# rvp-group/mrhash

Measured on AMD Instinct MI355X. Metric: depth frames/sec integrated (640x480), higher is better.
Workload: dtype f32; 1 GPU; replica-room0 stand-in 640x480, single-resolution hash TSDF integrate (alloc+compact+integrate+GC per frame, replica.cfg params), frames resident in HBM; frames_per_gpu=7880, parallelism=single GPU, live_blocks_end=39984, distinct_frames=200

## Files before the change

mrhash_amd/csrc/mrh_context.h:

```cpp
#pragma once

constexpr int kPipeRing = 6;

namespace {

thread_local std::string g_create_err;

struct EvPair {
  hipEvent_t a, b;
};

struct UpSlot {
  void* h = nullptr;
  void* d = nullptr;
  size_t cap = 0;
  hipEvent_t copied = nullptr;
  bool copied_rec = false;
  uint64_t last_seq = 0;
};
struct UpRing {
  UpSlot s[3];
  int cur = -1;
  hipStream_t stream = nullptr;
  hipEvent_t last_copy = nullptr;
  bool waited[2] = {false, false};
};

template <typename T>
struct HostVec {
  T* p = nullptr;
  T* dev = nullptr;
  bool pin = true;
  size_t n = 0, cap = 0;
  size_t span = 0, head = 0;
  HostVec() = default;
  HostVec(const HostVec&) = delete;
  HostVec& operator=(const HostVec&) = delete;
  ~HostVec() { release(); }
  void release() {
    if (!p) return;
    if (dev) (void) hipHostUnregister((void*) p);
    (void) munmap((void*) ((char*) p - head), span);
    p = nullptr; dev = nullptr; cap = 0; span = 0; head = 0;
  }
  T* data() { return p; }
  const T* data() const { return p; }
  size_t size() const { return n; }
  bool empty() const { return n == 0; }
  void clear() { n = 0; }
  const T& operator[](size_t i) const { return p[i]; }
  bool pin_pending = false;
  void map_(const size_t count, const bool touch) {
    release();
    const size_t want = count + count / 8;
    const size_t bytes = ((want * sizeof(T) + (2u << 20) - 1) >> 21) << 21;
    const size_t sp = bytes + (2u << 20);
    void* m = mmap(nullptr, sp, PROT_READ | PROT_WRITE, MAP_PRIVATE | MAP_ANONYMOUS, -1, 0);
    if (m == MAP_FAILED) throw std::bad_alloc();
    char* aligned = (char*) (((uintptr_t) m + (2u << 20) - 1) & ~(uintptr_t) ((2u << 20) - 1));
    (void) madvise(aligned, bytes, MADV_HUGEPAGE);
    if (touch) for (size_t o = 0; o < bytes; o += 4096) ((volatile char*) aligned)[o] = 0;
    span = sp;
    head = (size_t) (aligned - (char*) m);
    p = (T*) aligned;
    dev = nullptr;
    cap = bytes / sizeof(T);
  }
  void register_() {
    pin_pending = false;
    void* d = nullptr;
    const size_t bytes = cap * sizeof(T);
    if (hipHostRegister((void*) p, bytes, hipHostRegisterDefault) == hipSuccess && hipHostGetDevicePointer(&d, (void*) p, 0) == hipSuccess && d) {
      dev = (T*) d;
    } else {
      (void) hipGetLastError();
      (void) hipHostUnregister((void*) p);
      (void) hipGetLastError();
      dev = nullptr;
    }
  }
  void reserve_unpinned(const size_t count) {
    if (count <= cap) return;
    map_(count, true);
    pin_pending = pin;
    n = 0;
  }
  void resize_discard(size_t count) {
    if (count > cap) {
      map_(count, pin);
      pin_pending = false;
      if (pin) register_();
    } else if (pin_pending) {
      register_();
    }
    n = count;
  }
  void assign(const T* a, const T* b) {
    resize_discard((size_t) (b - a));
    if (n) memcpy(p, a, n * sizeof(T));
  }
};

struct FrameInputs {
  Cam cam;
  const float* d_depth; const uint8_t* d_rgb;
  int depth_rows, depth_cols, rgb_rows, rgb_cols;
  struct Ring { int cur; hipEvent_t last_copy; bool waited[2]; } ring[2];
};
struct DeferredFrame {
  bool on = false;
  int n_inval = 0;
  FrameInputs in;
};

enum FrameKind {
  FRAME_SERIAL,
  FRAME_PIPELINED,
  FRAME_FUSED_MR,
  FRAME_GENERAL,
};
struct FramePlan {
  FrameKind kind = FRAME_SERIAL;
  int max_num_frames = 0;
  bool starve_now = false;
  bool starve_fused = false;
  bool starve_in_pipe = false;
  bool gc_inline = false;
  bool safe_div = false, sph = false;
  float gc_thr = 0.f;
  int set = 0, zero_set = 0;
  int ring = 0, seq = 0;
  u32 stamp = 0;
  int tiles_x = 0, n_tiles = 0;
};
struct PendingBack {
  FramePlan plan;
  Cam cam; Fast f; Lists L;
  EvPair ev;
  uint64_t report_seq;
  bool count_zombies;
};

struct PipeState {
  hipStream_t stream_front = nullptr;
  hipEvent_t ev_front[kPipeRing] = {};
  int4* ring_vis[kPipeRing] = {}; int4* ring_bbox[kPipeRing] = {}; int4* ring_cfree[kPipeRing] = {}; float* ring_zmin[kPipeRing] = {};
  u32* want_ring = nullptr;
  int* h_levels = nullptr;
  uint2* dcx[kPipeRing] = {};
  size_t npix = 0;
  uint64_t fast_frames = 0;
  uint64_t seq = 0;
  uint64_t base = 0;
  int lazy_run = 0;
  bool zombies_possible = false;
  bool front_needs_sync = false;
  static constexpr int kPendMax = 3;
  PendingBack pendq[kPendMax];
  int npend = 0;
  bool last_frame_lazy = false;
  bool flushed_since_frame = false;
  int sync_streak = 0;
  u64* d_zfused = nullptr;
  size_t zfused_n = 0;
  bool zfused_clean[2] = {false, false};
  size_t zfused_clean_npix = 0;
  int zfused_next = 0;
};

}

struct mrh_ctx {
  mrh_params p;
  int device = 0;
  hipStream_t stream = nullptr;
  struct Owned { std::vector<void*> dev, pinned; std::vector<hipEvent_t> events; } owned;
  Cam cam;
  Map map;
  Tab tab;
  bool has_camera = false;
  bool spherical = false;
  UpRing up_depth, up_rgb;
  DeferredFrame deferred;
  int defer_uploads = 1;
  hipEvent_t frame_done[8] = {};
  hipEvent_t peek_done[8] = {};
  uint64_t frame_seq = 1;
  int* h_peek = nullptr;
  void* arena[3] = {nullptr, nullptr, nullptr};
  size_t arena_cap[3] = {0, 0, 0};
  uint64_t peek_seq[8] = {};
  bool peek_enabled = false;
  const float* d_depth = nullptr;
  const uint8_t* d_rgb = nullptr;
  int depth_rows = 0, depth_cols = 0, rgb_rows = 0, rgb_cols = 0;
  u32* d_decision = nullptr;
  u64* d_zbuf = nullptr;
  size_t zbuf_n = 0;
  bool starve_fused = true;
  bool starve_serial = false;
  uint64_t n_starve_fused = 0;
  int4* d_realloc = nullptr;
  int4* d_reint = nullptr;
  int* d_flag = nullptr;
  u64* d_upd_partials = nullptr;
  u32* d_misc = nullptr;
  float* d_rcp_w = nullptr;
  Fast fast;
  int pipe = 1;
  int pipe_grid = 1024;
  int pipe_uploads = 0;
  int pipe_period = 64;
  bool pipe_always_wait = false;
  int pipe_defer = 1;
  PipeState ps;
  FramePlan plan;
  uint64_t dbg_waits = 0;
  double dbg_spin_us = 0, dbg_api_us = 0; uint64_t dbg_lazy_frames = 0;
  int4* d_cfree = nullptr;
  float* d_cloud = nullptr; size_t cloud_n = 0;
  bool fast_summaries_stale = false;
  struct Lidar {
    float* d_points = nullptr;
    const float* d_points_cur = nullptr;
    size_t points_cap = 0, num_points = 0;
    float* d_normals = nullptr; size_t normals_cap = 0, num_normals = 0;
    bool have_cloud = false;
    int layout_hint = 0;
    int row_len = 0;
    uint64_t detect_n = 0;
    int detect_len = 0, detect_age = 0;
    int patch_log2 = 4;
    u32* d_pt_counts = nullptr; u32* d_pt_offsets = nullptr; size_t pt_cap = 0;
    u32* h_sorted_report = nullptr;
    u32 sorted_seq = 0;
    void* d_rec_keys[2] = {nullptr, nullptr}; float* d_rec_vals[2] = {nullptr, nullptr}; size_t rec_cap = 0, rec_key_bytes = 0;
    void* d_sort_tmp = nullptr; size_t sort_tmp_bytes = 0;
    Scan buckets = {};
    int use_buckets = 1;
    int buckets_scratch = 0;
    bool buckets_dirty = false;
    size_t buckets_rec_cap = 0, buckets_wg_cap = 0;
    u32* d_buckets_ctr = nullptr;
    u32 buckets_seq = 0;
    size_t buckets_lds_set = 0;
  } lidar;
  size_t qt_cap = 0;
  QSum* d_qt_sums = nullptr; u32* d_qt_flags = nullptr; u32* d_qt_unc = nullptr; u64* d_qt_marks = nullptr; u64* d_qt_pos = nullptr;
  mrh_splat_seed* d_qt_parked = nullptr; mrh_qtree_leaf* d_qt_leaves = nullptr;
  mrh_splat_seed* h_qt_seeds = nullptr; size_t qt_seed_cap = 0;
  u64* h_qt_out = nullptr;
  u64* d_qt_misc = nullptr;
  int qt_literal = 0;
  uint32_t qt_last_literal = 0;
  std::vector<mrh_qtree_leaf> qt_leaves;
  uint64_t qt_n_leaves = 0;
  bool qt_leaves_on_host = true;
  int mr_fused = 1;
  bool mr_next_general = true;
  bool mr_summaries_valid = false;
  bool refill_flag_valid = false;
  int mesh_on_host = 0;
  float* d_zmin = nullptr;
  u64* d_cnt_partials = nullptr;
  int fused_grid = 2048;
  int sweep_wgs_mr = 1024;
  int sweep_wgs = 128;
  int integrate_grid = 1024;
  int low_blocks_to_allocate = 0;
  uint64_t num_blocks = 0, slots = 0, max_triangles = 0;
  uint64_t frames = 0;
  int heap_descending = 0;
  int pending = 0;
  HostVec<mrh_triangle> tris;
  std::vector<mrh_block_desc> tri_blocks;
  std::vector<uint32_t> tri_counts;
  int tri_dev_n = 0;
  const int4* d_tri_sorted = nullptr;
  const u32* d_tri_counts = nullptr;
  u64* h_mc = nullptr;
  hipEvent_t ev_mc_total = nullptr;
  u32* d_mc_recs = nullptr; size_t mc_rec_cap = 0;
  uint64_t mc_rec_fallbacks = 0;
  HostVec<double> V, C;
  HostVec<int32_t> F;
  HostVec<float> V32, C32;
  HostVec<u32> stage_ctl;
  u32 stage_epoch = 0;
  void* mesh_clean_base = nullptr;
  size_t mesh_clean_words = 0;
  bool prewarm_on = true, prewarm_done = false;
  uint64_t n_extractions = 0;
  bool f64_link = false;
  int profile = 0;
  std::vector<EvPair> ev_pool;
  std::vector<EvPair> ev_pending;
  std::vector<EvPair> ev_pending_front;
  float sum_ms = 0.f, last_ms = 0.f;
  uint64_t n_ms = 0;
  float sum_front_ms = 0.f;
  uint64_t n_front_ms = 0;
  uint64_t prev_total_updated = 0, prev_inserted = 0, prev_freed = 0, total_compact = 0;
  uint64_t last_triangles = 0;
  int census_period = 64;
  int census_force = 0;
  uint64_t frames_since_census = 0;
  bool table_dirty = false;
  u32 flags_seen = 0, flags_deferred = 0, flags_peeked = 0;
  char* d_pack = nullptr; size_t pack_cap = 0;
  mrh_triangle* d_soup = nullptr; size_t soup_cap = 0, soup_n = 0;
  int4* d_halo = nullptr; size_t halo_cap = 0, halo_upper = 0;
  u32* d_taken = nullptr;
  hipEvent_t mc_ev[4] = {};
  float last_mc_count_ms = 0.f, last_mc_emit_ms = 0.f;
  uint64_t last_mc_blocks = 0;
  bool merge_on = false;
  mrh_triangle* d_acc = nullptr; size_t acc_cap = 0, acc_n = 0;
  mrh_comm* comm = nullptr;
  char* d_xsend = nullptr; size_t xsend_cap = 0;
  char* d_xrecv = nullptr; size_t xrecv_cap = 0;
  hipEvent_t comm_ev[5] = {};
  mrh_comm_phases comm_phases = {};
  std::vector<EvPair> comm_ev_pool, comm_ev_pending;
  char* d_ray = nullptr; size_t ray_cap = 0;
  char* h_ray = nullptr; size_t h_ray_cap = 0;
  struct Normals {
    NrmTab tab = {};
    size_t cap = 0;
    u64* d_ctr = nullptr;
    u32 seq = 0;
    bool dirty = false;
    int fold = 1;
    u64* h_ctr = nullptr;
    mrh_normals_info info = {};
    bool info_pending = false;
    float* h_out = nullptr; size_t h_out_cap = 0;
  } nrm;
  std::string err;
};

static int comm_allreduce_zbuf(mrh_ctx* c, mrh::u64* buf, size_t n);
static void comm_release(mrh_ctx* c);
static bool comm_matches_sharding(const mrh_ctx* c, int* comm_rank, int* comm_world);
namespace {
int strict_point(mrh_ctx* c);
int flush_deferred(mrh_ctx* c);
void main_stream_changed_map(mrh_ctx* c) { c->ps.front_needs_sync = true; }

int fail(mrh_ctx* c, int code, const char* fmt, ...) {
  char buf[512];
  va_list ap;
  va_start(ap, fmt);
  vsnprintf(buf, sizeof buf, fmt, ap);
  va_end(ap);
  if (c) c->err = buf;
  else g_create_err = buf;
  return code;
}

#define HIP_TRY(ctx, expr)                                                                                   \
  do {                                                                                                       \
    hipError_t e__ = (expr);                                                                                 \
    if (e__ != hipSuccess) return fail(ctx, MRH_ERR_DEVICE, "%s failed: %s (%s:%d)", #expr, hipGetErrorString(e__), __FILE__, __LINE__); \
  } while (0)

template <typename T>
struct DevBuf {
  T* p = nullptr;
  DevBuf() = default;
  DevBuf(const DevBuf&) = delete;
  DevBuf& operator=(const DevBuf&) = delete;
  ~DevBuf() { if (p) (void) hipFree(p); }
  hipError_t alloc(size_t n) { return hipMalloc((void**) &p, n * sizeof(T)); }
  operator T*() const { return p; }
};

template <typename T> hipError_t own(std::vector<void*>& ledger, T*& p, const hipError_t e) {
  if (e != hipSuccess) p = nullptr; else ledger.push_back((void*) p);
  return e;
}
template <typename T> hipError_t disown(std::vector<void*>& ledger, T*& p, hipError_t (*release)(void*)) {
  const auto it = std::find(ledger.begin(), ledger.end(), (void*) p);
  const hipError_t e = !p ? hipSuccess : it == ledger.end() ? hipErrorInvalidValue : release((void*) p);
  if (it != ledger.end()) { *it = ledger.back(); ledger.pop_back(); }
  p = nullptr;
  return e;
}
template <typename T> hipError_t dev_alloc(mrh_ctx* c, T*& p, const size_t bytes) { return own(c->owned.dev, p, hipMalloc((void**) &p, bytes)); }
template <typename T> hipError_t dev_free(mrh_ctx* c, T*& p) { return disown(c->owned.dev, p, hipFree); }
template <typename T> hipError_t pinned_alloc(mrh_ctx* c, T*& p, const size_t bytes) { return own(c->owned.pinned, p, hipHostMalloc((void**) &p, bytes, hipHostMallocDefault)); }
template <typename T> hipError_t pinned_free(mrh_ctx* c, T*& p) { return disown(c->owned.pinned, p, hipHostFree); }
hipError_t event_new(mrh_ctx* c, hipEvent_t& ev, const bool timing) {
  const hipError_t e = timing ? hipEventCreate(&ev) : hipEventCreateWithFlags(&ev, hipEventDisableTiming);
  if (e != hipSuccess) ev = nullptr; else c->owned.events.push_back(ev);
  return e;
}

struct GrowMember {
  void** p; size_t bytes;
  template <typename T> GrowMember(T*& q, size_t b) : p((void**) &q), bytes(b) {}
};
int regrow_all(mrh_ctx* c, size_t& cap, const size_t cap_new, std::initializer_list<GrowMember> members, const bool sync = true) {
  cap = 0;
  if (sync) HIP_TRY(c, hipStreamSynchronize(c->stream));
  for (const GrowMember& m : members) HIP_TRY(c, dev_free(c, *m.p));
  for (const GrowMember& m : members) {
    const hipError_t e = dev_alloc(c, *m.p, m.bytes);
    if (e == hipSuccess) continue;
    for (const GrowMember& f : members) (void) dev_free(c, *f.p);
    return fail(c, MRH_ERR_DEVICE, "hipMalloc of %zu bytes failed: %s", m.bytes, hipGetErrorString(e));
  }
  cap = cap_new;
  return MRH_OK;
}
template <typename T>
int regrow(mrh_ctx* c, T*& p, size_t& cap, const size_t cap_new, const size_t bytes, const bool sync = true) {
  return cap_new <= cap ? MRH_OK : regrow_all(c, cap, cap_new, {{p, bytes}}, sync);
}
template <typename T>
int regrow_keep(mrh_ctx* c, T*& p, size_t& cap, const size_t cap_new, const size_t bytes_new, const size_t keep_bytes) {
  if (cap_new <= cap) return MRH_OK;
  T* grown = nullptr;
  HIP_TRY(c, dev_alloc(c, grown, bytes_new));
  struct Drop { mrh_ctx* c; T*& p; ~Drop() { (void) dev_free(c, p); } } drop{c, grown};
  if (p && keep_bytes) HIP_TRY(c, hipMemcpyAsync(grown, p, keep_bytes, hipMemcpyDeviceToDevice, c->stream));
  HIP_TRY(c, hipStreamSynchronize(c->stream));
  std::swap(p, grown); cap = cap_new;
  return MRH_OK;
}
template <typename T>
int regrow_pinned(mrh_ctx* c, T*& p, size_t& cap, const size_t cap_new, const size_t bytes) {
  if (cap_new <= cap) return MRH_OK;
  cap = 0;
  (void) pinned_free(c, p);
  HIP_TRY(c, pinned_alloc(c, p, bytes));
  cap = cap_new;
  return MRH_OK;
}

uint64_t next_pow2(uint64_t v) {
  uint64_t r = 1;
  while (r < v) r <<= 1;
  return r;
}

void free_all(mrh_ctx* c) {
  if (!c) return;
  (void) hipSetDevice(c->device);
  hipStream_t* streams[4] = {&c->up_depth.stream, &c->up_rgb.stream, &c->ps.stream_front, &c->stream};
  for (hipStream_t* s : streams) if (*s) (void) hipStreamSynchronize(*s);
  comm_release(c);
  for (hipEvent_t e : c->owned.events) (void) hipEventDestroy(e);
  for (void* p : c->owned.pinned) (void) hipHostFree(p);
  for (void* p : c->owned.dev) (void) hipFree(p);
  c->owned = {};
  for (hipStream_t* s : streams) if (*s) { (void) hipStreamDestroy(*s); *s = nullptr; }
}

void reset_pipe_counters(mrh_ctx* c) {
  PipeState& ps = c->ps;
  for (int i = 0; i < ps.npend; i++) if (ps.pendq[i].ev.a) c->ev_pool.push_back(ps.pendq[i].ev);
  ps.npend = 0;
  ps.fast_frames = 0;
  ps.seq = ps.base = 0;
  ps.lazy_run = 0;
  ps.zombies_possible = false;
  ps.front_needs_sync = false;
}

int init_buffers(mrh_ctx* c) {
  hipStream_t s = c->stream;
  c->mr_next_general = true;
  c->refill_flag_valid = false;
  c->mr_summaries_valid = false;
  if (c->ps.stream_front) HIP_TRY(c, hipStreamSynchronize(c->ps.stream_front));
  reset_pipe_counters(c);
  if (c->ps.h_levels) { c->ps.h_levels[0] = (int) c->num_blocks - 1; c->ps.h_levels[1] = 0; c->ps.h_levels[2] = -1; }
  if (c->ps.want_ring) HIP_TRY(c, hipMemsetAsync(c->ps.want_ring, 0, (size_t) kPipeRing * c->slots * sizeof(u32), s));
  const Tab& t = c->tab;
  k_init_table<<<1024, 256, 0, s>>>(t.keys, c->slots);
  k_init_heap<<<1024, 256, 0, s>>>(t.heap_fine, (u32) c->num_blocks, c->heap_descending);
  HIP_TRY(c, hipMemsetAsync(t.vals, 0, c->slots * sizeof(u32), s));
  HIP_TRY(c, hipMemsetAsync(t.desc_fine, 0, c->num_blocks * sizeof(int4), s));
  if (t.multi_res) HIP_TRY(c, hipMemsetAsync(t.desc_coarse, 0, c->num_blocks * 8 * sizeof(int4), s));
  HIP_TRY(c, hipMemsetAsync(t.pool, 0, c->num_blocks * (size_t) kFineBytes, s));
  int h_ctr[CTR_COUNT];
  memset(h_ctr, 0, sizeof h_ctr);
  h_ctr[CTR_HEAP_FINE] = (int) c->num_blocks - 1;
  h_ctr[CTR_HEAP_COARSE] = -1;
  HIP_TRY(c, hipMemcpyAsync(t.ctr, h_ctr, sizeof h_ctr, hipMemcpyHostToDevice, s));
  HIP_TRY(c, hipMemsetAsync(t.prof, 0, PROF_COUNT * sizeof(u64), s));
  HIP_TRY(c, hipMemsetAsync(c->d_upd_partials, 0, (size_t) c->integrate_grid * sizeof(u64), s));
  HIP_TRY(c, hipMemsetAsync(c->d_cnt_partials, 0, (size_t) 32768 * 4 * sizeof(u64), s));
  HIP_TRY(c, hipStreamSynchronize(s));
  c->frames = 0;
  c->frames_since_census = 0;
  c->table_dirty = false;
  c->flags_seen = c->flags_deferred = c->flags_peeked = 0;
  c->halo_upper = 0;
  c->prev_total_updated = c->prev_inserted = c->prev_freed = c->total_compact = 0;
  c->sum_ms = c->last_ms = 0.f;
  c->n_ms = 0;
  c->sum_front_ms = 0.f;
  c->n_front_ms = 0;
  c->tris.clear(); c->V.clear(); c->C.clear(); c->F.clear();
  c->last_triangles = 0;
  return MRH_OK;
}

int create_checks(const mrh_params* p) {
  if (p->abi_version != MRH_ABI_VERSION) return fail(nullptr, MRH_ERR_INVALID_ARG, "mrh_create: abi_version mismatch");
  if (!(p->virtual_voxel_size > 0.f)) return fail(nullptr, MRH_ERR_INVALID_ARG, "mrh_create: virtual_voxel_size must be > 0");
  if (!(p->sdf_truncation >= 0.f) || !(p->sdf_truncation_scale >= 0.f))
    return fail(nullptr, MRH_ERR_INVALID_ARG, "mrh_create: sdf_truncation and sdf_truncation_scale must be >= 0");
  if (p->voxel_extents_scale != 0 && p->voxel_extents_scale != 1)
    return fail(nullptr, MRH_ERR_UNSUPPORTED, "mrh_create: voxel_extents_scale != 1 is incoherent in the reference (vhu.cuh:90-92 vs 138-140)");
  int ndev = 0;
  if (hipGetDeviceCount(&ndev) != hipSuccess || ndev <= 0) return fail(nullptr, MRH_ERR_NO_DEVICE, "mrh_create: no HIP device visible");
  if (p->device_id < 0 || p->device_id >= ndev) return fail(nullptr, MRH_ERR_INVALID_ARG, "mrh_create: device_id %d out of range (%d devices)", p->device_id, ndev);
  if (p->shard_count > 1 && (p->shard_rank < 0 || p->shard_rank >= p->shard_count))
    return fail(nullptr, MRH_ERR_INVALID_ARG, "mrh_create: shard_rank out of range");
  return MRH_OK;
}

int size_map(mrh_ctx* c, const mrh_params* p) {
  c->p = *p;
  if (c->p.integration_weight_max == 0) c->p.integration_weight_max = 255;
  if (c->p.voxel_extents_scale == 0) c->p.voxel_extents_scale = 1;
  if (c->p.shard_count < 1) c->p.shard_count = 1;
  c->device = p->device_id;
  memset(&c->tab, 0, sizeof c->tab); memset(&c->cam, 0, sizeof c->cam); memset(&c->fast, 0, sizeof c->fast);
  HIP_TRY(c, hipSetDevice(c->device));
  HIP_TRY(c, hipStreamCreateWithFlags(&c->stream, hipStreamNonBlocking));
  size_t free_b = 0, total_b = 0;
  HIP_TRY(c, hipMemGetInfo(&free_b, &total_b));
  const double to_alloc = (double) free_b * 0.70;
  c->num_blocks = p->num_sdf_blocks ? p->num_sdf_blocks : (uint64_t) ((to_alloc * 0.70) / (12.0 * 512.0));
  if (c->num_blocks >= (1ull << 28)) c->num_blocks = (1ull << 28) - 1;
  c->max_triangles = p->max_triangles ? p->max_triangles : (uint64_t) ((to_alloc * 0.25) / 72.0);
  c->slots = std::max<uint64_t>(1024, next_pow2(p->hash_slots ? p->hash_slots : 4 * c->num_blocks));
  c->low_blocks_to_allocate = (int) ((float) c->num_blocks * 0.1f);
  c->fast.zlist_cap = (u32) c->num_blocks;
  Tab& t = c->tab;
  t.slot_mask = (u32) (c->slots - 1); t.max_probe = 512; t.cap_blocks = (u32) c->num_blocks;
  t.multi_res = p->sdf_var_threshold > 0.f ? 1u : 0u;
  Map& m = c->map;
  m.vs = p->virtual_voxel_size; m.trunc = p->sdf_truncation; m.trunc_scale = p->sdf_truncation_scale;
  m.var_threshold = p->sdf_var_threshold; m.mc_threshold = p->marching_cubes_threshold; m.min_weight_threshold = p->min_weight_threshold;
  m.weight_sample = p->integration_weight_sample & 0xFF; m.weight_max = c->p.integration_weight_max & 0xFF;
  m.shard_rank = c->p.shard_rank; m.shard_count = c->p.shard_count;
  m.shard_chunk_log2 = (p->shard_chunk_log2 > 0 && p->shard_chunk_log2 < 16) ? p->shard_chunk_log2 : 3;
  return MRH_OK;
}

int alloc_map(mrh_ctx* c) {
  Tab& t = c->tab;
  const size_t nb = c->num_blocks, list_cap = nb * (t.multi_res ? 9 : 1);
  HIP_TRY(c, dev_alloc(c, t.keys, c->slots * sizeof(u64)));                HIP_TRY(c, dev_alloc(c, t.vals, c->slots * sizeof(u32)));
  HIP_TRY(c, dev_alloc(c, t.heap_fine, (nb + 1) * sizeof(u32)));           HIP_TRY(c, dev_alloc(c, t.desc_fine, nb * sizeof(int4)));
  if (t.multi_res) {
    HIP_TRY(c, dev_alloc(c, t.heap_coarse, (nb * 8 + 9) * sizeof(u32)));   HIP_TRY(c, dev_alloc(c, t.desc_coarse, nb * 8 * sizeof(int4)));
    HIP_TRY(c, dev_alloc(c, c->d_realloc, nb * sizeof(int4)));             HIP_TRY(c, dev_alloc(c, c->d_reint, nb * sizeof(int4)));
    HIP_TRY(c, dev_alloc(c, c->fast.summary_c, nb * 8 * sizeof(uint2)));
  }
  HIP_TRY(c, dev_alloc(c, t.pool, nb * (size_t) kFineBytes));
  HIP_TRY(c, dev_alloc(c, t.compact, list_cap * sizeof(int4)));            HIP_TRY(c, dev_alloc(c, c->d_decision, list_cap * sizeof(u32)));
  HIP_TRY(c, dev_alloc(c, t.ctr, CTR_COUNT * sizeof(int)));                HIP_TRY(c, dev_alloc(c, t.prof, PROF_COUNT * sizeof(u64)));
  HIP_TRY(c, dev_alloc(c, c->d_flag, sizeof(int)));                        HIP_TRY(c, dev_alloc(c, c->d_misc, 4 * sizeof(u32)));
  HIP_TRY(c, dev_alloc(c, c->d_upd_partials, (size_t) c->integrate_grid * sizeof(u64)));
  HIP_TRY(c, dev_alloc(c, c->d_cnt_partials, (size_t) 32768 * 4 * sizeof(u64)));
  HIP_TRY(c, dev_alloc(c, c->fast.summary, nb * sizeof(uint2)));           HIP_TRY(c, dev_alloc(c, c->fast.bbox, list_cap * sizeof(int4)));
#ifdef MRH_TRACE
  HIP_TRY(c, dev_alloc(c, c->fast.trace, nb * 8 * sizeof(u64)));
  HIP_TRY(c, hipMemset(c->fast.trace, 0, nb * 8 * sizeof(u64)));
#endif
  HIP_TRY(c, dev_alloc(c, c->d_cfree, list_cap * sizeof(int4)));           HIP_TRY(c, dev_alloc(c, c->d_zmin, list_cap * sizeof(float)));
  return MRH_OK;
}

int probe_arithmetic(mrh_ctx* c) {
  Map& m = c->map;
  const bool dbg = getenv("MRH_DEBUG") != nullptr;
  const u32 init = 1u << 23;
  u32 first_bad = 0;
  if (hipMemcpy(c->d_misc, &init, sizeof init, hipMemcpyHostToDevice) != hipSuccess) first_bad = 1;
  k_block_shift_limit<<<(1 << 23) / 256, 256, 0, c->stream>>>(m.vs, c->d_misc);
  if (hipStreamSynchronize(c->stream) != hipSuccess || hipMemcpy(&first_bad, c->d_misc, sizeof first_bad, hipMemcpyDeviceToHost) != hipSuccess) first_bad = 1;
  int lim = 1;
  while ((u32) (lim << 1) <= first_bad && lim < (1 << 22)) lim <<= 1;
  m.block_shift_limit = first_bad <= 1 ? 0 : lim;
  if (dbg) fprintf(stderr, "[mrhash_hip] voxel->block is a shift for |v| < %d (first mismatch at %u, voxel size %g)\n", m.block_shift_limit, first_bad, (double) m.vs);
  auto rn_reciprocal = [](float b) {
    const float c0 = (float) (1.0 / (double) b);
    float best = c0;
    double err = std::fabs(1.0 - (double) c0 * (double) b);
    for (float t : {std::nextafter(c0, 0.f), std::nextafter(c0, INFINITY)}) {
      const double e = std::fabs(1.0 - (double) t * (double) b);
      if (e < err) { err = e; best = t; }
    }
    return best;
  };
  std::vector<float> dev(kRcpWeightEntries, 0.f);
  bool ok = dev_alloc(c, c->d_rcp_w, dev.size() * sizeof(float)) == hipSuccess;
  if (ok) {
    k_rcp_weights<<<(kRcpWeightEntries + 255) / 256, 256, 0, c->stream>>>(c->d_rcp_w);
    ok = hipStreamSynchronize(c->stream) == hipSuccess && hipMemcpy(dev.data(), c->d_rcp_w, dev.size() * sizeof(float), hipMemcpyDeviceToHost) == hipSuccess;
  }
  int w_bad = ok ? 0 : 1;
  for (int w = 1; ok && w <= 510; w++) w_bad += dev[w] != rn_reciprocal((float) w);
  m.wsum_two_steps = w_bad ? 1 : 0;
  const float half_vs = m.vs / 2;
  m.r_half_vs = rn_reciprocal(half_vs);
  u32 bad = 1;
  if (hipMemset(c->d_misc, 0, sizeof(u32)) == hipSuccess) {
    k_check_div_cr<<<4096, 256, 0, c->stream>>>(half_vs, m.r_half_vs, c->d_misc);
    if (hipStreamSynchronize(c->stream) != hipSuccess || hipMemcpy(&bad, c->d_misc, sizeof bad, hipMemcpyDeviceToHost) != hipSuccess) bad = 1;
  }
  m.half_vs_two_steps = bad ? 1 : 0;
  if (dbg) fprintf(stderr, "[mrhash_hip] division by vs / 2 with one residual step: %u mismatches over the working range -> %s; refined reciprocals of the weight sums: %d not correctly rounded\n", bad, bad ? "two steps" : "one step", w_bad);
  return MRH_OK;
}

template <typename T> void env_onoff(const char* name, T& v) { if (const char* g = getenv(name)) v = atoi(g) ? 1 : 0; }
inline bool env_present(const char* name) { return getenv(name) != nullptr; }
template <typename T> void env_int(const char* name, const int64_t lo, const int64_t hi, T& v) {
  if (const char* g = getenv(name)) { const int x = atoi(g); if (x >= lo && x <= hi) v = (T) x; }
}

void read_switches(mrh_ctx* c) {
  constexpr int64_t kIntMax = 0x7FFFFFFF;
  env_int("MRH_FUSED_GRID", 1, 32768, c->fused_grid);
  env_onoff("MRH_DEFER_UPLOADS", c->defer_uploads);
  env_onoff("MRH_PIPE", c->pipe);
  env_onoff("MRH_STARVE_FUSED", c->starve_fused);
  c->starve_serial = env_present("MRH_STARVE_SERIAL");
  c->pipe_always_wait = env_present("MRH_PIPE_ALWAYS_WAIT");
  env_int("MRH_PIPE_GRID", 1, 32768, c->pipe_grid);
  env_int("MRH_PIPE_DEFER", 1, PipeState::kPendMax - 1, c->pipe_defer);
  env_onoff("MRH_PIPE_UPLOADS", c->pipe_uploads);
  env_int("MRH_PIPE_PERIOD", 1, kIntMax, c->pipe_period);
  env_int("MRH_SWEEP_WGS", 1, 4096, c->sweep_wgs);
  env_int("MRH_SWEEP_WGS_MR", 1, 4096, c->sweep_wgs_mr);
  env_onoff("MRH_MR_FUSED", c->mr_fused);
  env_int("MRH_ZLIST_CAP", 1, (int64_t) c->num_blocks - 1, c->fast.zlist_cap);
  int safe_div = 0, rehash_off = 0;
  env_onoff("MRH_SAFE_DIV", safe_div);
  if (safe_div) c->map.half_vs_two_steps = 1;
  c->heap_descending = env_present("MRH_DEBUG_HEAP_DESCENDING") ? 1 : 0;
  env_onoff("MRH_PREWARM", c->prewarm_on);
  env_onoff("MRH_MESH_HOST", c->mesh_on_host);
  env_onoff("MRH_MESH_F64_LINK", c->f64_link);
  c->V.pin = c->C.pin = c->f64_link;
  env_onoff("MRH_QTREE_LITERAL", c->qt_literal);
  env_int("MRH_SCAN_ROW_LEN", -kIntMax - 1, kIntMax, c->lidar.layout_hint);
  env_int("MRH_SCAN_PATCH_LOG2", 0, 8, c->lidar.patch_log2);
  env_onoff("MRH_LIDAR_BUCKETS", c->lidar.use_buckets);
  env_onoff("MRH_NORMALS_FOLD", c->nrm.fold);
  if (const char* g = getenv("MRH_SCAN_SEQ_START")) c->lidar.buckets_seq = (u32) strtoul(g, nullptr, 0);
  env_int("MRH_REHASH_PERIOD", 1, kIntMax, c->census_period);
  env_onoff("MRH_REHASH_FORCE", c->census_force);
  env_onoff("MRH_REHASH_OFF", rehash_off);
  if (rehash_off) c->census_period = -1;
}

}
```

mrhash_amd/csrc/mrh_fast.h:

```cpp
#pragma once

#include "mrh_kernels.h"

namespace mrh {

constexpr int CTR_CULLED = 12;
constexpr int CTR_FREED_EARLY = 13;
constexpr float kFltMax = 3.402823466e+38f;
constexpr int kTileMaxPx = 576;

struct Fast {
  uint2* dcx;
  uint2* summary;
  u32 zlist_cap;
  int4* bbox;
  uint2* summary_c;
  u32* want;
  int4* zlist;
#ifdef MRH_TRACE
  u64* trace;
#endif
};

#ifdef MRH_TRACE
__device__ __forceinline__ u64 trace_now() {
  u64 t;
  asm volatile("s_waitcnt lgkmcnt(0)\n\ts_memrealtime %0\n\ts_waitcnt lgkmcnt(0)" : "=s"(t) : : "memory");
  return t;
}
#define MRH_TS(slot) do { if (lane == 0) f.trace[(size_t) e * 8 + (slot)] = trace_now(); } while (0)
constexpr size_t kTraceFront = 32768;
#define MRH_TSF(slot) do { if (threadIdx.x == 0) f.trace[(kTraceFront + blockIdx.x) * 8 + (slot)] = trace_now(); } while (0)
#else
#define MRH_TS(slot) do { } while (0)
#define MRH_TSF(slot) do { } while (0)
#endif

__device__ __forceinline__ void wave_free_block(const Tab& t, const int4 ent, const int lane) {
  const u32 H = (u32) ent.w;
  if (lane == 0) {
    u64 key;
    pack_key(mki3(ent.x, ent.y, ent.z), key);
    hash_erase(t, key);
    const int idx = atomicAdd(&t.ctr[CTR_HEAP_FINE], 1);
    t.heap_fine[idx + 1] = H;
    t.desc_fine[H].w = 0;
  }
  uint4* p = (uint4*) (t.pool + (size_t) H * kFineBytes);
  const uint4 z = make_uint4(0, 0, 0, 0);
#pragma unroll
  for (int k = 0; k < kFineBytes / 16 / kWave; k++) p[k * kWave + lane] = z;
}




struct Proj4 {
  float pcz[4];
  int row[4], col[4];
  u32 mask;
};
template <bool SPH>
__device__ __forceinline__ bool proj_ok(const Cam& c, const Proj4& P, const int k) {
  const bool depth_ok = SPH ? !(P.pcz[k] < c.min_depth || P.pcz[k] > c.max_depth) : !(P.pcz[k] <= c.min_depth || P.pcz[k] > c.max_depth);
  return depth_ok && (u32) P.row[k] < (u32) c.rows && (u32) P.col[k] < (u32) c.cols;
}

__device__ __forceinline__ Proj4 project4(const Cam& c, const Map& m, const int4 ent, const int q) {
  Proj4 P;
  const int x0 = ent.x * kBlockSide + (q & 1) * 4;
  const int y = ent.y * kBlockSide + ((q >> 1) & 7);
  const int z = ent.z * kBlockSide + (q >> 4);
  const float py = y * m.vs, pz = z * m.vs;
  const float a1 = c.Ri[1] * py, a2 = c.Ri[2] * pz;
  const float b1 = c.Ri[4] * py, b2 = c.Ri[5] * pz;
  const float c1 = c.Ri[7] * py, c2 = c.Ri[8] * pz;
  P.mask = 0;
#pragma unroll
  for (int k = 0; k < 4; k++) {
    const float px = (x0 + k) * m.vs;
    const float X = ((c.Ri[0] * px + a1) + a2) + c.ti[0];
    const float Y = ((c.Ri[3] * px + b1) + b2) + c.ti[1];
    const float Z = ((c.Ri[6] * px + c1) + c2) + c.ti[2];
    P.pcz[k] = Z;
    const bool depth_ok = !(Z <= c.min_depth || Z > c.max_depth);
    const float rz = rcp_refined(Z);
    const int row = f2i_hw((div_rr(c.fy * Y, Z, rz) + c.cy) + 0.5f);
    const int col = f2i_hw((div_rr(c.fx * X, Z, rz) + c.cx) + 0.5f);
    const bool ok = depth_ok && (u32) row < (u32) c.rows && (u32) col < (u32) c.cols;
    P.row[k] = row;
    P.col[k] = col;
    P.mask |= ok ? (1u << k) : 0u;
  }
  return P;
}

__device__ __forceinline__ Proj4 project4_sph(const Cam& c, const Map& m, const int4 ent, const int q) {
  Proj4 P;
  const int x0 = ent.x * kBlockSide + (q & 1) * 4;
  const int y = ent.y * kBlockSide + ((q >> 1) & 7);
  const int z = ent.z * kBlockSide + (q >> 4);
  const float py = y * m.vs, pz = z * m.vs;
  const float a1 = c.Ri[1] * py, a2 = c.Ri[2] * pz;
  const float b1 = c.Ri[4] * py, b2 = c.Ri[5] * pz;
  const float c1 = c.Ri[7] * py, c2 = c.Ri[8] * pz;
  P.mask = 0;
#pragma unroll
  for (int k = 0; k < 4; k++) {
    const float px = (x0 + k) * m.vs;
    const float X = ((c.Ri[0] * px + a1) + a2) + c.ti[0];
    const float Y = ((c.Ri[3] * px + b1) + b2) + c.ti[1];
    const float Z = ((c.Ri[6] * px + c1) + c2) + c.ti[2];
    const float range = sqrtf(X * X + Y * Y + Z * Z);
    P.pcz[k] = range;
    const bool depth_ok = !(range < c.min_depth || range > c.max_depth);
    const float az = mrh_atan2f(Y, X);
    const float el = mrh_asinf(Z / range);
    const int row = f2i_hw((c.fy * el + c.cy) + 0.5f);
    const int col = f2i_hw((c.fx * az + c.cx) + 0.5f);
    const bool ok = depth_ok && (u32) row < (u32) c.rows && (u32) col < (u32) c.cols;
    P.row[k] = row;
    P.col[k] = col;
    P.mask |= ok ? (1u << k) : 0u;
  }
  return P;
}

struct Sdf4 {
  v2f sd[2], trn[2];
};
template <typename PT>
__device__ __forceinline__ void update4(const Cam& c, const Map& m, const PT& P, const bool (&ok)[4], const float (&d)[4], Sdf4& g,
                                        bool (&upd)[4]) {
#pragma unroll
  for (int k = 0; k < 4; k += 2) {
    const v2f dd = mk2(d[k], d[k + 1]);
    g.trn[k >> 1] = splat2(m.trunc) + splat2(m.trunc_scale) * dd;
    g.sd[k >> 1] = dd - mk2(P.pcz[k], P.pcz[k + 1]);
  }
#pragma unroll
  for (int k = 0; k < 4; k++) {
    const bool depth_bad = (d[k] == 0.f) || (d[k] > c.max_int_dist);
    const float sdf = (k & 1) ? g.sd[k >> 1].y : g.sd[k >> 1].x;
    const float trn = (k & 1) ? g.trn[k >> 1].y : g.trn[k >> 1].x;
    upd[k] = ok[k] && !(depth_bad || sdf <= -trn);
  }
}
template <typename PT>
__device__ __forceinline__ u32 update_mask4(const Cam& c, const Map& m, const PT& P, const float (&d)[4]) {
  Sdf4 g;
  bool upd[4];
  const bool ok[4] = {(P.mask & 1u) != 0, (P.mask & 2u) != 0, (P.mask & 4u) != 0, (P.mask & 8u) != 0};
  update4(c, m, P, ok, d, g, upd);
  return (upd[0] ? 1u : 0u) | (upd[1] ? 2u : 0u) | (upd[2] ? 4u : 0u) | (upd[3] ? 8u : 0u);
}

template <bool SAFEDIV, bool KEEP_SS>
__device__ __forceinline__ void blend4(const Map& m, const Sdf4& g, const bool (&upd)[4], const u32 (&cpx)[4], float (&s)[4], u32 (&w)[4],
                                       float (&ss)[4]) {
  const u32 w1 = (u32) (m.weight_sample & 0xFF);
  const u32 wmax = (u32) (m.weight_max & 0xFF);
  const v2f half_vs = splat2(m.vs / 2), rh = splat2(m.r_half_vs), w1f = splat2((float) w1);
  constexpr bool two = SAFEDIV, two_w = SAFEDIV;
#pragma unroll
  for (int k = 0; k < 4; k += 2) {
    const v2f trn = g.trn[k >> 1];
    v2f sd = g.sd[k >> 1];
    sd = mk2(__builtin_amdgcn_fmed3f(sd.x, -trn.x, trn.x), __builtin_amdgcn_fmed3f(sd.y, -trn.y, trn.y));
    const v2f s0 = mk2(s[k], s[k + 1]);
    const u32 old0 = w[k], old1 = w[k + 1];
    const u32 w00 = old0 >> 24, w01 = old1 >> 24;
    const v2f curr_mean = mk2(w00 > 0 ? s0.x : sd.x, w01 > 0 ? s0.y : sd.y);
    const v2f delta = div_cr2(sd - curr_mean, half_vs, rh, two);
    const v2f w0f = mk2((float) w00, (float) w01);
    const v2f wsum = w0f + w1f;
    const v2f sn = div_cr2(s0 * w0f + sd * w1f, wsum, rcp_refined2(wsum), two_w);
    const v2f delta2 = div_cr2(sd - sn, half_vs, rh, two);
    const v2f sq = splat2(0.f) + delta * delta2;
#pragma unroll
    for (int j = 0; j < 2; j++) {
      const u32 old = j ? old1 : old0, w0 = j ? w01 : w00;
      const u32 c1x = cpx[k + j] & 0x00FFFFFFu;
      const u32 c0x = (w0 == 0) ? c1x : (old & 0x00FFFFFFu);
      const u32 rgbn = (c0x | c1x) - (((c0x ^ c1x) >> 1) & 0x007F7F7Fu);
      const u32 wn = (w0 + w1) < wmax ? (w0 + w1) : wmax;
      const bool u = upd[k + j];
      s[k + j] = u ? (j ? sn.y : sn.x) : s[k + j];
      w[k + j] = u ? (rgbn | (wn << 24)) : w[k + j];
      ss[k + j] = (u || !KEEP_SS) ? (j ? sq.y : sq.x) : ss[k + j];
    }
  }
}

__device__ __forceinline__ float pixel_reach(const Cam& c, const Map& m, const float d) {
  const bool rejected = (d == 0.f) || (d > c.max_int_dist);
  return rejected ? 0.f : (d > 0.f ? d + get_truncation(d, m.trunc, m.trunc_scale) : kFltMax);
}
struct TileRegs {
  float dv[4];
  u32 cv[4];
};
__device__ __forceinline__ float tile_inv_w(const int4 bb) { return __builtin_amdgcn_rcpf((float) bb.z); }
__device__ __forceinline__ void tile_issue(const Cam& c, const Fast& f, const int4 bb, const int lane, TileRegs& tr) {
  const int npx = bb.z * bb.w;
  if (npx <= 0) return;
  const float inv_w = tile_inv_w(bb);
#pragma unroll
  for (int j = 0; j < 4; j++) {
    const int p = min(lane + 64 * j, npx - 1);
    const int r = (int) (((float) p + 0.5f) * inv_w);
    const int cc = p - r * bb.z;
    const u32 g = (u32) (__mul24(bb.y + r, c.cols) + bb.x + cc);
    const uint2 v = f.dcx[g];
    tr.dv[j] = __uint_as_float(v.x);
    tr.cv[j] = v.y;
  }
}
__device__ __forceinline__ float tile_commit(const Cam& c, const Map& m, const Fast& f, const int4 bb, const int lane, uint2* tile,
                                             const TileRegs& tr) {
  const int npx = bb.z * bb.w;
  float reach = 0.f;
  if (npx <= 0) return reach;
#pragma unroll
  for (int j = 0; j < 4; j++) {
    const int p = lane + 64 * j;
    if (p < npx) tile[p] = make_uint2(__float_as_uint(tr.dv[j]), tr.cv[j]);
    reach = __uint_as_float(umax_(__float_as_uint(reach), __float_as_uint(pixel_reach(c, m, tr.dv[j]))));
  }
  if (npx > 256) {
    const float inv_w = tile_inv_w(bb);
#pragma unroll 1
    for (int p0 = 256 + lane; p0 < npx; p0 += 128) {
      float dv[2];
      u32 cv[2];
#pragma unroll
      for (int j = 0; j < 2; j++) {
        const int p = min(p0 + 64 * j, npx - 1);
        const int r = (int) (((float) p + 0.5f) * inv_w);
        const int cc = p - r * bb.z;
        const u32 g = (u32) (__mul24(bb.y + r, c.cols) + bb.x + cc);
        const uint2 v = f.dcx[g];
        dv[j] = __uint_as_float(v.x);
        cv[j] = v.y;
      }
#pragma unroll
      for (int j = 0; j < 2; j++) {
        const int p = p0 + 64 * j;
        if (p < npx) tile[p] = make_uint2(__float_as_uint(dv[j]), cv[j]);
        reach = __uint_as_float(umax_(__float_as_uint(reach), __float_as_uint(pixel_reach(c, m, dv[j]))));
      }
    }
  }
  return reach;
}

template <int NB>
__device__ __forceinline__ void tile_lookup(const Fast& f, const int cols, const int4 bb, const uint2* tile, const Proj4 (&P)[NB],
                                            const bool (&ok)[NB][4], float (&d)[NB][4], u32 (&cpx)[NB][4]) {
  bool miss[NB][4], any_miss = false;
  u32 li[NB][4];
#pragma unroll
  for (int b = 0; b < NB; b++)
#pragma unroll
    for (int k = 0; k < 4; k++) {
      const u32 lr = (u32) (P[b].row[k] - bb.y), lc = (u32) (P[b].col[k] - bb.x);
      const bool in = lr < (u32) bb.w && lc < (u32) bb.z;
      li[b][k] = in ? __umul24(lr, (u32) bb.z) + lc : 0u;
      miss[b][k] = !in && ok[b][k];
      any_miss = any_miss || miss[b][k];
    }
#pragma unroll
  for (int b = 0; b < NB; b++)
#pragma unroll
    for (int k = 0; k < 4; k++) {
      const uint2 px = tile[li[b][k]];
      d[b][k] = __uint_as_float(px.x);
      cpx[b][k] = px.y;
    }
  if (__ballot(any_miss)) {
#pragma unroll
    for (int b = 0; b < NB; b++)
#pragma unroll
      for (int k = 0; k < 4; k++)
        if (miss[b][k]) {
          const u32 pix = (u32) (__mul24(P[b].row[k], cols) + P[b].col[k]);
          const uint2 v = f.dcx[pix];
          d[b][k] = __uint_as_float(v.x);
          cpx[b][k] = v.y;
        }
  }
}

__global__ __launch_bounds__(256) void k_count_updates(const Cam c, const Map m, const Tab t, const Fast f, u64* __restrict__ partials,
                                                       const int merged_set, const int4* __restrict__ vis, const int4* __restrict__ cfree, const u32 want_stamp, const int zombies) {
  const int nvis = merged_set >= 0 ? t.ctr[merged_set] : t.ctr[CTR_COMPACT];
  const int lane = threadIdx.x & 63;
  const int gw = blockIdx.x * 4 + (threadIdx.x >> 6);
  const int nw = gridDim.x * 4;
  u32 cnt = 0, zskip = 0, zcul = 0;
  for (int e = gw; e < nvis; e += nw) {
    const int4 ent = vis[e];
    if (zombies && (f.summary[ent.w].y & 0x80000000u)) {
      int wanted = 0;
      if (lane == 0) {
        u64 key;
        pack_key(mki3(ent.x, ent.y, ent.z), key);
        const int slot = hash_find(t, key);
        wanted = (slot >= 0 && f.want[slot] == want_stamp) ? 1 : 0;
      }
      if (!__builtin_amdgcn_readfirstlane(wanted)) { zskip++; continue; }
    }
#pragma unroll
    for (int b = 0; b < 2; b++) {
      const Proj4 P = c.model ? project4_sph(c, m, ent, lane + 64 * b) : project4(c, m, ent, lane + 64 * b);
      float d[4];
#pragma unroll
      for (int k = 0; k < 4; k++) d[k] = __uint_as_float(f.dcx[((P.mask >> k) & 1u) ? (u32) (__mul24(P.row[k], c.cols) + P.col[k]) : 0u].x);
      cnt += __popc(update_mask4(c, m, P, d));
    }
  }
  if (zombies && merged_set >= 0) {
    const int ncf = t.ctr[merged_set + 2];
    for (int e = gw * 64 + lane; e < ncf; e += nw * 64) {
      const int4 ent = cfree[e];
      if (f.summary[ent.w].y & 0x80000000u) {
        u64 key;
        pack_key(mki3(ent.x, ent.y, ent.z), key);
        const int slot = hash_find(t, key);
        if (!(slot >= 0 && f.want[slot] == want_stamp)) zcul++;
      }
    }
    for (int off = 32; off > 0; off >>= 1) zcul += __shfl_xor(zcul, off);
    zskip += zcul;
  }
  for (int off = 32; off > 0; off >>= 1) cnt += __shfl_xor(cnt, off);
  if (lane == 0) {
    partials[gw] += (u64) cnt;
    if (zskip) atomicAdd((unsigned long long*) &t.prof[PROF_COMPACT], (unsigned long long) (0ull - (u64) zskip));
    if (gw == 0)
      atomicAdd((unsigned long long*) &t.prof[PROF_COMPACT], merged_set >= 0 ? (unsigned long long) (nvis + t.ctr[merged_set + 1] + t.ctr[merged_set + 2])
                                                                             : (unsigned long long) (nvis + t.ctr[CTR_CULLED] + t.ctr[CTR_FREED_EARLY]));
  }
}

}
```

mrhash_amd/csrc/mrh_fast2.h:

```cpp
#pragma once

#include "mrh_pipe.h"

namespace mrh {

constexpr int CTR_SET0 = 32;
constexpr int kListSets = 6;
constexpr u32 kZombieBit = 0x80000000u;

struct Lists {
  int4* vis;
  int4* bbox;
  int4* cfree;
  float* zmin;
  u32 cap;
};

__device__ __forceinline__ int desc_w(u32 stamp) { return (int) (1u | (stamp << 1)); }

struct FrontShared {
  u64 set[kRayCap];
  u64 list[kRayCap];
  u32 count, inserted;
  int nvis, nfree, nkeep, bv, bf;
};

__device__ __forceinline__ int commit_block(const Tab& t, const Fast& f, const int slot, const int heap_idx, const i3 b, const u32 stamp,
                                            const int hwm_at_start) {
  if (heap_idx < 0) {
    publish_without_storage(t, slot, CTR_HEAP_FINE);
    return -1;
  }
  const u32 H = t.heap_fine[heap_idx];
  t.vals[slot] = H;
  t.desc_fine[H] = make_int4(b.x, b.y, b.z, desc_w(stamp));
  f.summary[H] = make_uint2(0x7F7FFFFFu, 0u);
  if ((int) H >= hwm_at_start) atomicMax(&t.ctr[CTR_HWM_FINE], (int) H + 1);
  return (int) H;
}

template <bool SPH = false>
__device__ __forceinline__ bool tile_rays(const Cam& c, const Map& m, uint2* __restrict__ dcx, const float* __restrict__ depth,
                                          const uint8_t* __restrict__ rgb, const int tiles_x, const int tile_id, FrontShared& sh, float& d_out) {
  constexpr int NT = 256;
  const int tid = threadIdx.x;
  for (int i = tid; i < kRayCap; i += NT) sh.set[i] = kKeyEmpty;
  if (tid == 0) { sh.count = 0; sh.inserted = 0; }
  __syncthreads();
  const int ty = tile_id / tiles_x, tx = tile_id - ty * tiles_x;
  const int row = ty * kRayTile + (tid >> 4), col = tx * kRayTile + (tid & 15);
  bool slow = false;
  d_out = 0.f;
  if (row < c.rows && col < c.cols) {
    const size_t pix = (size_t) row * c.cols + col;
    float d = depth[pix];
    if (d <= c.min_depth || d > c.max_depth) d = 0.f;
    if (SPH && d != 0.f) d = get_depth(c, inverse_projection_m(c, (u32) row, (u32) col, d));
    d_out = d;
    const uint8_t* px = rgb + pix * 3;
    dcx[pix] = make_uint2(__float_as_uint(d), (u32) px[0] | ((u32) px[1] << 8) | ((u32) px[2] << 16));
    const RayState ray = ray_setup<SPH>(c, m, row, col, d);
    if (ray.valid) {
      if (!ray_keys_in_range(ray)) {
        slow = true;
      } else {
        slow = !walk_ray_lean(m, ray, [&](const i3 cur, const u64 key) {
          u32 s = (u32) __mul24(cur.z, 5851) + (u32) __mul24(cur.y, 73) + (u32) cur.x;
          s = (s ^ (s >> 7)) & (kRayCap - 1);
#pragma unroll 1
          for (int p = 0; p < kSetProbe; p++) {
            const u64 old = atomicCAS(&sh.set[s], kKeyEmpty, key);
            if (old == kKeyEmpty) { sh.list[atomicAdd(&sh.count, 1u)] = key; return true; }
            if (old == key) return true;
            s = (s + 1) & (kRayCap - 1);
          }
          return false;
        });
      }
    }
  }
  __syncthreads();
  return slow;
}

template <bool PROFILE, bool MARK, bool SPH = false>
__device__ __forceinline__ void tile_slow_pixel(const Cam& c, const Map& m, const Tab& t, const Fast& f, const Lists& L, const int row, const int col,
                                                const float d, const u32 stamp, const int cs, const int hwm0) {
  walk_ray<SPH>(c, m, t, row, col, d, [&](const i3 cur, const u64 key) {
    if (MARK) {
      const int s0 = hash_find(t, key);
      if (s0 >= 0) { f.want[s0] = stamp; return; }
    }
    if (!(SPH ? block_in_frustum_approx_m(c, m.vs, cur) : block_in_frustum_approx(c, m.vs, cur))) return;
    const int slot = hash_insert(t, key);
    if (slot == -2) atomicOr((u32*) &t.ctr[CTR_ERROR], ERR_TABLE);
    if (slot < 0) return;
    const int H = commit_block(t, f, slot, atomicSub(&t.ctr[CTR_HEAP_FINE], 1), cur, stamp, hwm0);
    if (H < 0) return;
    const int li = atomicAdd(&t.ctr[cs + 0], 1);
    L.vis[li] = make_int4(cur.x, cur.y, cur.z, H);
    L.bbox[li] = make_int4(0, 0, 0, 0);
    if (PROFILE) atomicAdd(&t.prof[PROF_INSERTED], 1ull);
  });
}

template <bool MARK, bool SPH = false>
__device__ __forceinline__ u32 wave_insert_keys(const Cam& c, const Map& m, const Tab& t, const Fast& f, const Lists& L, const u64 key,
                                                const u32 stamp, const int cs, const int hwm0) {
  const bool active = key != kKeyEmpty;
  const i3 b = active ? unpack_key(key) : mki3(0, 0, 0);
  bool won = false;
  int slot = -1;
  int claim;
  u64 claim_val;
  if (active) {
    const int found = hash_find_claim(t, key, claim, claim_val);
    if (found >= 0) {
      if (MARK) f.want[found] = stamp;
    } else if (SPH ? block_in_frustum_approx_m(c, m.vs, b) : block_in_frustum_approx(c, m.vs, b)) {
      slot = hash_insert_at(t, key, claim, claim_val);
      if (slot == -2) atomicOr((u32*) &t.ctr[CTR_ERROR], ERR_TABLE);
      won = slot >= 0;
    }
  }
  const u64 ballot = __ballot(won);
  u32 inserted = 0;
  if (ballot) {
    const int leader = __ffsll((long long) ballot) - 1;
    int hb = 0;
    if ((int) lane_id() == leader) hb = atomicSub(&t.ctr[CTR_HEAP_FINE], __popcll(ballot));
    hb = __shfl(hb, leader);
    const int hidx = hb - __popcll(ballot & lanemask_lt());
    const u64 ok = __ballot(won && hidx >= 0);
    int lb = 0;
    if (ok && (int) lane_id() == __ffsll((long long) ok) - 1) lb = atomicAdd(&t.ctr[cs + 0], __popcll(ok));
    int H = -1;
    if (won) H = commit_block(t, f, slot, hidx, b, stamp, hwm0);
    if (ok) {
      const int lead2 = __ffsll((long long) ok) - 1;
      lb = __shfl(lb, lead2);
      if (H >= 0) {
        const int idx = lb + __popcll(ok & lanemask_lt());
        L.vis[idx] = make_int4(b.x, b.y, b.z, H);
        L.bbox[idx] = make_int4(0, 0, 0, 0);
        inserted = 1;
      }
    }
  }
  return inserted;
}

template <bool PROFILE, bool MARK, bool SPH = false>
__device__ __forceinline__ void front_tile(const Cam& c, const Map& m, const Tab& t, const Fast& f, const Lists& L,
                                           const float* __restrict__ depth, const uint8_t* __restrict__ rgb, const int tiles_x,
                                           const int tile_id, const u32 stamp, const int cs, FrontShared& sh) {
  constexpr int NT = 256;
  const int tid = threadIdx.x;
  const int hwm0 = t.ctr[CTR_HWM_FINE];
  MRH_TSF(1);
  float d;
  const bool slow = tile_rays<SPH>(c, m, f.dcx, depth, rgb, tiles_x, tile_id, sh, d);
  MRH_TSF(3);
  if (slow) {
    const int ty = tile_id / tiles_x, tx = tile_id - ty * tiles_x;
    tile_slow_pixel<PROFILE, MARK, SPH>(c, m, t, f, L, ty * kRayTile + (tid >> 4), tx * kRayTile + (tid & 15), d, stamp, cs, hwm0);
  }
  const int n = (int) sh.count;
  u32 my_inserted = 0;
#pragma unroll 1
  for (int base = 0; base < n; base += NT) {
    const int i = base + tid;
    my_inserted += wave_insert_keys<MARK, SPH>(c, m, t, f, L, i < n ? sh.list[i] : kKeyEmpty, stamp, cs, hwm0);
  }
  MRH_TSF(4);
#ifdef MRH_TRACE
  if (tid == 0) {
    u32 hw;
    asm volatile("s_getreg_b32 %0, hwreg(HW_REG_HW_ID)" : "=s"(hw));
    u32 xcc;
    asm volatile("s_getreg_b32 %0, hwreg(HW_REG_XCC_ID)" : "=s"(xcc));
    f.trace[(kTraceFront + blockIdx.x) * 8 + 7] = (u64) n;
    f.trace[(kTraceFront + blockIdx.x) * 8 + 5] = (u64) hw | ((u64) xcc << 32);
  }
#endif
  if (PROFILE) {
    if (my_inserted) atomicAdd(&sh.inserted, my_inserted);
    __syncthreads();
    if (tid == 0 && sh.inserted) atomicAdd(&t.prof[PROF_INSERTED], (u64) sh.inserted);
  }
}

template <bool MULTI, bool DEFER = false, bool SPH = false>
__device__ __forceinline__ void front_sweep(const Cam& c, const Map& m, const Tab& t, const Fast& f, const Lists& L, const u32 stamp,
                                            const int cs, const int gc_on, const float trunc_threshold, const int sw, const int n_sweep,
                                            FrontShared& sh) {
  constexpr int NT = 256;
  const int tid = threadIdx.x;
  const int hwm = t.ctr[CTR_HWM_FINE];
  int4* st_vis = (int4*) sh.list;
  int4* st_free = (int4*) sh.set;
  constexpr int kStVis = kRayCap * 8 / 32, kStFree = kRayCap * 8 / 16;
  if (tid == 0) { sh.nvis = 0; sh.nfree = 0; sh.nkeep = 0; }
  __syncthreads();
  auto flush = [&]() {
    __syncthreads();
    if (tid == 0) {
      sh.bv = sh.nvis ? atomicAdd(&t.ctr[cs + 0], sh.nvis) : 0;
      sh.bf = sh.nfree ? atomicAdd(&t.ctr[cs + 2], sh.nfree) : 0;
    }
    __syncthreads();
    for (int i = tid; i < sh.nvis; i += NT) {
      const int4 pk = st_vis[2 * i + 1];
      L.vis[sh.bv + i] = st_vis[2 * i];
      L.bbox[sh.bv + i] = make_int4(pk.x, pk.y, pk.z & 0xFFFF, (int) ((u32) pk.z >> 16));
      L.zmin[sh.bv + i] = __int_as_float(pk.w);
    }
    for (int i = tid; i < sh.nfree; i += NT) L.cfree[sh.bf + i] = st_free[i];
    __syncthreads();
    if (tid == 0) { sh.nvis = 0; sh.nfree = 0; }
    __syncthreads();
  };
  const int grp = tid >> 2;
  const int sub = tid & 3;
  auto sweep_range = [&](const int4* __restrict__ descs, const uint2* __restrict__ sums, const int total, const u32 valbit) {
  const int chunk = (((total + n_sweep - 1) / n_sweep) + 63) & ~63;
  const int lo = sw * chunk, hi = min(total, lo + chunk);
  int4 d_next = make_int4(0, 0, 0, 0);
  uint2 sm_next = make_uint2(0, 0);
  if (lo + grp < hi) { d_next = descs[lo + grp]; sm_next = sums[lo + grp]; }
  for (int base = lo; base < hi; base += 64) {
    const int i = base + grp;
    const int4 d = d_next;
    const uint2 sm = sm_next;
    if (i + 64 < hi) { d_next = descs[i + 64]; sm_next = sums[i + 64]; }
    const bool live = i < hi && (d.w & 1) && ((u32) d.w >> 1) != stamp;
    if (__ballot(live) != 0) {
      int any_approx = 0;
      float zmin = kFltMax, zmax = -kFltMax, umin = kFltMax, umax = -kFltMax, vmin = kFltMax, vmax = -kFltMax;
#pragma unroll
      for (int h = 0; h < 2; h++) {
        const int corner = sub + 4 * h;
        const i3 v = mki3(d.x * kBlockSide + ((corner & 4) ? 7 : 0), d.y * kBlockSide + ((corner & 2) ? 7 : 0), d.z * kBlockSide + ((corner & 1) ? 7 : 0));
        const f3 pc = se3_apply(c.Ri, c.ti, voxel_to_world(m.vs, v));
        int r, cc;
        any_approx |= (SPH ? project_point_m<true>(c, pc, r, cc) : project_point<true>(c, pc, r, cc)) ? 1 : 0;
        zmin = fminf(zmin, pc.z); zmax = fmaxf(zmax, pc.z);
        if (!SPH && pc.z >= 0.05f) {
          const float u = c.fx * pc.x / pc.z + c.cx;
          const float w = c.fy * pc.y / pc.z + c.cy;
          umin = fminf(umin, u); umax = fmaxf(umax, u);
          vmin = fminf(vmin, w); vmax = fmaxf(vmax, w);
        }
      }
#pragma unroll
      for (int off = 1; off < 4; off <<= 1) {
        any_approx |= __shfl_xor(any_approx, off);
        zmin = fminf(zmin, __shfl_xor(zmin, off)); zmax = fmaxf(zmax, __shfl_xor(zmax, off));
        umin = fminf(umin, __shfl_xor(umin, off)); umax = fmaxf(umax, __shfl_xor(umax, off));
        vmin = fminf(vmin, __shfl_xor(vmin, off)); vmax = fmaxf(vmax, __shfl_xor(vmax, off));
      }
      if (sub == 0 && live && any_approx) {
        bool cull = !SPH && ((zmax <= c.min_depth - 1e-3f) || (zmin > c.max_depth + 1e-3f));
        if (!SPH && !cull && zmin >= 0.05f) cull = umax < -3.f || umin > (float) c.cols + 1.f || vmax < -3.f || vmin > (float) c.rows + 1.f;
        const int4 e = make_int4(d.x, d.y, d.z, (int) ((u32) i | valbit));
        if (!cull) {
          int4 bb = make_int4(0, 0, 0, 0);
          if (!SPH && zmin >= 0.05f) {
            int c0 = f2i_hw(floorf(umin + 0.5f)) - 1, c1 = f2i_hw(floorf(umax + 0.5f)) + 1;
            int r0 = f2i_hw(floorf(vmin + 0.5f)) - 1, r1 = f2i_hw(floorf(vmax + 0.5f)) + 1;
            c0 = c0 < 0 ? 0 : c0; r0 = r0 < 0 ? 0 : r0;
            c1 = c1 > c.cols - 1 ? c.cols - 1 : c1; r1 = r1 > c.rows - 1 ? c.rows - 1 : r1;
            const int bw = c1 - c0 + 1, bh = r1 - r0 + 1;
            if (bw > 0 && bh > 0 && bw * bh <= kTileMaxPx) bb = make_int4(c0, r0, bw | (bh << 16), __float_as_int(zmin));
          }
          const int k2 = atomicAdd(&sh.nvis, 1);
          st_vis[2 * k2] = e;
          st_vis[2 * k2 + 1] = bb;
        } else {
          bool collect = false;
          if (gc_on) {
            collect = DEFER || (__uint_as_float(sm.x) >= trunc_threshold) || (sm.y == 0u);
          }
          if (collect) st_free[atomicAdd(&sh.nfree, 1)] = e;
          else atomicAdd(&sh.nkeep, 1);
        }
      }
    }
    __syncthreads();
    if (sh.nvis > kStVis - 64 || sh.nfree > kStFree - 64) flush();
  }
  };
  sweep_range(t.desc_fine, f.summary, hwm, 0u);
  if (MULTI) sweep_range(t.desc_coarse, f.summary_c, 8 * hwm, kValCoarseBit);
  flush();
  if (tid == 0 && sh.nkeep) atomicAdd(&t.ctr[cs + 1], sh.nkeep);
  MRH_TSF(4);
#ifdef MRH_TRACE
  if (tid == 0) f.trace[(kTraceFront + blockIdx.x) * 8 + 7] = (u64) (hwm / n_sweep) | (1ull << 63);
#endif
}

__device__ __forceinline__ void front_refill(const Tab& t, const int low_blocks_to_allocate, const int* __restrict__ flag, const int wg) {
  if (*flag == 0) return;
  const int i = wg * 256 + (int) threadIdx.x;
  if (i >= low_blocks_to_allocate) return;
  const int addr_high = atomicSub(&t.ctr[CTR_HEAP_FINE], 1);
  if (addr_high < 0) { atomicAdd(&t.ctr[CTR_HEAP_FINE], 1); atomicOr((u32*) &t.ctr[CTR_ERROR], ERR_POOL); return; }
  const u32 H = t.heap_fine[addr_high];
  atomicMax(&t.ctr[CTR_HWM_FINE], (int) H + 1);
  const int addr_low = atomicAdd(&t.ctr[CTR_HEAP_COARSE], 8);
  for (int idx = 1; idx <= 8; idx++) t.heap_coarse[addr_low + idx] = H * 8 + 8 - idx;
}

template <bool PROFILE, bool MULTI, bool LAZY = false, bool SPH = false>
__global__ __launch_bounds__(256) void k_front(const Cam c, const Map m, const Tab t, const Fast f, const Lists L,
                                               const float* __restrict__ depth, const uint8_t* __restrict__ rgb, const int tiles_x,
                                               const int n_tiles, const u32 stamp, const int set, const int gc_on,
                                               const float trunc_threshold, const int n_refill, const int low_blocks_to_allocate,
                                               const int* __restrict__ refill_flag) {
  __shared__ FrontShared sh;
  const int cs = CTR_SET0 + 4 * set;
  const int n_sweep = (int) gridDim.x - n_tiles - n_refill;
  MRH_TSF(0);
  if (MULTI && (int) blockIdx.x >= n_sweep + n_tiles) front_refill(t, low_blocks_to_allocate, refill_flag, (int) blockIdx.x - n_sweep - n_tiles);
  else if ((int) blockIdx.x >= n_sweep) front_tile<PROFILE, LAZY, SPH>(c, m, t, f, L, depth, rgb, tiles_x, (int) blockIdx.x - n_sweep, stamp, cs, sh);
  else front_sweep<MULTI, LAZY, SPH>(c, m, t, f, L, stamp, cs, gc_on, trunc_threshold, (int) blockIdx.x, n_sweep, sh);
}

__device__ __forceinline__ int4 wave_bbox(const Cam& c, const float vs, const int4 ent, const int lane, float& zmin_out) {
  const int corner = lane & 7;
  const i3 v = mki3(ent.x * kBlockSide + ((corner & 4) ? 7 : 0), ent.y * kBlockSide + ((corner & 2) ? 7 : 0), ent.z * kBlockSide + ((corner & 1) ? 7 : 0));
  const f3 pc = se3_apply(c.Ri, c.ti, voxel_to_world(vs, v));
  float zmin = pc.z;
  float umin = c.fx * pc.x / pc.z + c.cx, umax = umin;
  float vmin = c.fy * pc.y / pc.z + c.cy, vmax = vmin;
#pragma unroll
  for (int off = 1; off < 8; off <<= 1) {
    zmin = fminf(zmin, __shfl_xor(zmin, off));
    umin = fminf(umin, __shfl_xor(umin, off)); umax = fmaxf(umax, __shfl_xor(umax, off));
    vmin = fminf(vmin, __shfl_xor(vmin, off)); vmax = fmaxf(vmax, __shfl_xor(vmax, off));
  }
  int4 bb = make_int4(0, 0, 0, 0);
  if (zmin >= 0.05f) {
    int c0 = f2i_hw(floorf(umin + 0.5f)) - 1, c1 = f2i_hw(floorf(umax + 0.5f)) + 1;
    int r0 = f2i_hw(floorf(vmin + 0.5f)) - 1, r1 = f2i_hw(floorf(vmax + 0.5f)) + 1;
    c0 = c0 < 0 ? 0 : c0; r0 = r0 < 0 ? 0 : r0;
    c1 = c1 > c.cols - 1 ? c.cols - 1 : c1; r1 = r1 > c.rows - 1 ? c.rows - 1 : r1;
    const int bw = c1 - c0 + 1, bh = r1 - r0 + 1;
    if (bw > 0 && bh > 0 && bw * bh <= kTileMaxPx) bb = make_int4(c0, r0, bw, bh);
  }
  zmin_out = __shfl(zmin, 0);
  return make_int4(__shfl(bb.x, 0), __shfl(bb.y, 0), __shfl(bb.z, 0), __shfl(bb.w, 0));
}

typedef int v4i_ __attribute__((ext_vector_type(4)));
__device__ __forceinline__ void load_entry_scalar(const Lists& L, const int e, int4& ent, int4& bb, float& zmin) {
  v4i_ a, b;
  int z;
  const u32 off16 = (u32) e * 16u, off4 = (u32) e * 4u;
  asm volatile("s_load_dwordx4 %0, %3, %6\n\ts_load_dwordx4 %1, %4, %6\n\ts_load_dword %2, %5, %7\n\ts_waitcnt lgkmcnt(0)"
               : "=&s"(a), "=&s"(b), "=&s"(z)
               : "s"(L.vis), "s"(L.bbox), "s"(L.zmin), "s"(off16), "s"(off4)
               : "memory");
  ent = make_int4(a.x, a.y, a.z, a.w);
  bb = make_int4(b.x, b.y, b.z, b.w);
  zmin = __int_as_float(z);
}

__device__ __forceinline__ void wave_free_coarse(const Tab& t, const int4 ent, const int lane, u32* __restrict__ deferred) {
  const u32 u = (u32) ent.w & ~kValCoarseBit;
  if (lane == 0) {
    u64 key;
    pack_key(mki3(ent.x, ent.y, ent.z), key);
    hash_erase(t, key);
    t.desc_coarse[u].w = 0;
    deferred[atomicAdd(&t.ctr[CTR_NREINT], 1)] = u;
  }
  u32* p = (u32*) (t.pool + (size_t) (u >> 3) * kFineBytes + (size_t) (u & 7) * kCoarseBytes);
#pragma unroll
  for (int k = 0; k < kCoarseBytes / 4 / kWave; k++) p[k * kWave + lane] = 0u;
}
__device__ __forceinline__ void wave_free_any(const Tab& t, const int4 ent, const int lane, u32* __restrict__ deferred) {
  if ((u32) ent.w & kValCoarseBit) wave_free_coarse(t, ent, lane, deferred);
  else wave_free_block(t, ent, lane);
}

template <bool VARIANCE>
__device__ __forceinline__ bool coarse_block(const Cam& c, const Map& m, const Tab& t, const Fast& f, const float* __restrict__ depth,
                                             const uint8_t* __restrict__ rgb, const int4 ent, const int lane, const int first_n,
                                             const float trunc_threshold) {
  const u32 val = (u32) ent.w;
  const u32 u = val & ~kValCoarseBit;
  const VoxPtr vp = vox_ptr(t, val);
  const int v = lane;
  float sd = vp.sdf[v], sq = vp.sumsq[v];
  u32 rw = vp.rgbw[v];
  if (v < first_n) {
    const i3 pi = mki3(ent.x * kBlockSide + 2 * (v & 3), ent.y * kBlockSide + 2 * ((v >> 2) & 3), ent.z * kBlockSide + 2 * (v >> 4));
    if (integrate_voxel<VARIANCE>(c, m, depth, rgb, pi, &sd, &sq, &rw)) { vp.sdf[v] = sd; vp.sumsq[v] = sq; vp.rgbw[v] = rw; }
  }
  const u32 wk = rw >> 24;
  const float mn = __uint_as_float(wave_min_u32(umin_(0x7F7FFFFFu, wk != 0 ? (__float_as_uint(sd) & 0x7FFFFFFFu) : 0xFFFFFFFFu)));
  const u32 mx = wave_max_u32(wk);
  if (lane == 0) f.summary_c[u] = make_uint2(__float_as_uint(mn), mx);
  return mn >= trunc_threshold || mx == 0;
}

__device__ __forceinline__ bool variance_says_coarsen(const Map& m, const uint2* __restrict__ sv, const int lane) {
  float local_sum_sq = 0.f, local_weight = 0.f;
  const int gx = (lane % 4) * 2, gy = ((lane / 4) % 4) * 2, gz = (lane / 16) * 2;
#pragma unroll
  for (int dz = 0; dz < 2; ++dz)
#pragma unroll
    for (int dy = 0; dy < 2; ++dy)
#pragma unroll
      for (int dx = 0; dx < 2; ++dx) {
        const uint2 e = sv[(gz + dz) * 64 + (gy + dy) * 8 + (gx + dx)];
        const u32 w = e.y >> 24;
        if (w > 0) { local_sum_sq += __uint_as_float(e.x); local_weight += (float) w; }
      }
  for (int stride = 32; stride > 0; stride >>= 1) {
    const float os = __shfl_down(local_sum_sq, stride);
    const float ow = __shfl_down(local_weight, stride);
    if (lane < stride) { local_sum_sq += os; local_weight += ow; }
  }
  int coarsen = 0;
  if (lane == 0 && !(local_weight < 2)) {
    const double avg_var = (double) (local_sum_sq / (local_weight - 1));
    if ((local_weight - 1) > 1e-6f && avg_var > 0.f && avg_var < (double) m.var_threshold) coarsen = 1;
  }
  return __shfl(coarsen, 0) != 0;
}

__device__ __forceinline__ void wave_zombify(const Tab& t, const Fast& f, const int4 ent, const int lane) {
  const u32 H = (u32) ent.w;
  if (lane == 0) {
    f.summary[H] = make_uint2(0x7F7FFFFFu, kZombieBit);
    const int zi = atomicAdd(&t.ctr[CTR_ZOMBIES], 1);
    if ((u32) zi < f.zlist_cap) f.zlist[zi] = ent;
  }
  uint4* p = (uint4*) (t.pool + (size_t) H * kFineBytes);
  const uint4 z = make_uint4(0, 0, 0, 0);
#pragma unroll
  for (int k = 0; k < kFineBytes / 16 / kWave; k++) p[k * kWave + lane] = z;
}
__device__ __forceinline__ bool zombie_wanted(const Tab& t, const Fast& f, const int4 ent, const u32 want_stamp, const int lane) {
  int wanted = 0;
  if (lane == 0) {
    u64 key;
    pack_key(mki3(ent.x, ent.y, ent.z), key);
    const int slot = hash_find(t, key);
    wanted = (slot >= 0 && f.want[slot] == want_stamp) ? 1 : 0;
  }
  return __builtin_amdgcn_readfirstlane(wanted) != 0;
}

template <bool FREE, bool PROFILE, bool MULTI, bool SAFEDIV, int LZ = 0, bool SPH = false>
__device__ __forceinline__ void back_range(const Cam& c, const Map& m, const Tab& t, const Fast& f, const Lists& L,
                                           const float trunc_threshold, const int n, const int gw, const int nw, const int lane,
                                           uint2* tile, const float* __restrict__ depth_raw, const uint8_t* __restrict__ rgb_raw,
                                           u32* __restrict__ deferred, const u32 want_stamp = 0) {
  static_assert(!(MULTI && LZ), "multi-resolution maps are not pipelined");
  static_assert(!(MULTI && SPH), "multi-resolution maps under the spherical model take the general kernels");
  for (int e = __builtin_amdgcn_readfirstlane(gw); e < n; e += nw) {
    MRH_TS(0);
    int4 ent, bb;
    float zmin;
    load_entry_scalar(L, e, ent, bb, zmin);
    if (MULTI && ((u32) ent.w & kValCoarseBit)) {
      const bool collect = coarse_block<true>(c, m, t, f, depth_raw, rgb_raw, ent, lane, kCoarseVoxels, trunc_threshold);
      if (FREE && collect) {
        wave_free_coarse(t, ent, lane, deferred);
        if (PROFILE && lane == 0) atomicAdd(&t.prof[PROF_FREED], 1ull);
      }
      continue;
    }
    const u32 H = (u32) ent.w;
    float4* ps = (float4*) (t.pool + (size_t) H * kFineBytes);
    float4* pq = ps + 128;
    uint4* pw = (uint4*) (ps + 256);
    uint2 sm0 = make_uint2(0u, 0u);
    if (LZ) sm0 = f.summary[H];
    float4 S[2];
    uint4 W[2];
#pragma unroll
    for (int b = 0; b < 2; b++) { S[b] = ps[lane + 64 * b]; W[b] = pw[lane + 64 * b]; }
    float4 Q[2];
    if (MULTI) {
#pragma unroll
      for (int b = 0; b < 2; b++) Q[b] = pq[lane + 64 * b];
    }
    if (!SPH && bb.z == 0) bb = wave_bbox(c, m.vs, ent, lane, zmin);
    Proj4 P[2];
    float d[2][4];
    u32 cpx[2][4];
    MRH_TS(1);
    TileRegs tr;
    tile_issue(c, f, bb, lane, tr);
#pragma unroll
    for (int b = 0; b < 2; b++) P[b] = SPH ? project4_sph(c, m, ent, lane + 64 * b) : project4(c, m, ent, lane + 64 * b);
    if (LZ && (sm0.y & kZombieBit)) {
      if (!zombie_wanted(t, f, ent, want_stamp, lane)) {
        if (lane == 0) atomicAdd(&t.ctr[CTR_ZSKIP], 1);
        continue;
      }
      sm0 = make_uint2(0x7F7FFFFFu, 0u);
      if (lane == 0) f.summary[H] = sm0;
      if (PROFILE && lane == 0) atomicAdd(&t.prof[PROF_INSERTED], 1ull);
    }
    const float reach = tile_commit(c, m, f, bb, lane, tile, tr);
    const bool skip = bb.z != 0 && __ballot(!(reach + 1e-4f <= zmin)) == 0;
    float mn;
    u32 mx;
#ifdef MRH_TRACE
    u32 trace_upd = 0;
#endif
    if (skip) {
      const uint2 sm = LZ ? sm0 : f.summary[H];
      mn = __uint_as_float(sm.x);
      mx = sm.y;
    } else {
      MRH_TS(2);
      __builtin_amdgcn_fence(__ATOMIC_RELEASE, "wavefront");
      __builtin_amdgcn_wave_barrier();
      __builtin_amdgcn_fence(__ATOMIC_ACQUIRE, "wavefront");
      MRH_TS(3);
      bool ok[2][4];
#pragma unroll
      for (int b = 0; b < 2; b++)
#pragma unroll
        for (int k = 0; k < 4; k++) ok[b][k] = proj_ok<SPH>(c, P[b], k);
      tile_lookup<2>(f, c.cols, bb, tile, P, ok, d, cpx);
      __builtin_amdgcn_wave_barrier();
      MRH_TS(4);
      u32 mnb = 0x7F7FFFFFu;
      mx = 0;
#pragma unroll
      for (int b = 0; b < 2; b++) {
        const int q = lane + 64 * b;
        float s[4] = {S[b].x, S[b].y, S[b].z, S[b].w};
        u32 w[4] = {W[b].x, W[b].y, W[b].z, W[b].w};
        float ss[4] = {0.f, 0.f, 0.f, 0.f};
        if (MULTI) { ss[0] = Q[b].x; ss[1] = Q[b].y; ss[2] = Q[b].z; ss[3] = Q[b].w; }
        Sdf4 g;
        bool upd[4];
        update4(c, m, P[b], ok[b], d[b], g, upd);
        const bool any = upd[0] || upd[1] || upd[2] || upd[3], all = upd[0] && upd[1] && upd[2] && upd[3];
#ifdef MRH_TRACE
        trace_upd += (u32) upd[0] + (u32) upd[1] + (u32) upd[2] + (u32) upd[3];
#endif
        blend4<SAFEDIV, MULTI>(m, g, upd, cpx[b], s, w, ss);
        if (MULTI) {
          W[b] = make_uint4(w[0], w[1], w[2], w[3]);
          Q[b] = make_float4(ss[0], ss[1], ss[2], ss[3]);
        }
        if (any) {
          ps[q] = make_float4(s[0], s[1], s[2], s[3]);
          pw[q] = make_uint4(w[0], w[1], w[2], w[3]);
          if (all) {
            pq[q] = make_float4(ss[0], ss[1], ss[2], ss[3]);
          } else {
            float* pqs = (float*) (pq + q);
#pragma unroll
            for (int k = 0; k < 4; k++)
              if (upd[k]) pqs[k] = ss[k];
          }
        }
#pragma unroll
        for (int k = 0; k < 4; k++) {
          const u32 wk = w[k] >> 24;
          const u32 ab = __float_as_uint(s[k]) & 0x7FFFFFFFu;
          mnb = umin_(mnb, wk != 0 ? ab : 0xFFFFFFFFu);
          mx = umax_(mx, wk);
        }
      }
      mn = __uint_as_float(wave_min_u32(mnb));
      mx = wave_max_u32(mx);
      MRH_TS(5);
      if (MULTI) {
        __builtin_amdgcn_wave_barrier();
        uint2* sv = tile;
#pragma unroll
        for (int b = 0; b < 2; b++) {
          const int q = lane + 64 * b;
          sv[q * 4 + 0] = make_uint2(__float_as_uint(Q[b].x), W[b].x);
          sv[q * 4 + 1] = make_uint2(__float_as_uint(Q[b].y), W[b].y);
          sv[q * 4 + 2] = make_uint2(__float_as_uint(Q[b].z), W[b].z);
          sv[q * 4 + 3] = make_uint2(__float_as_uint(Q[b].w), W[b].w);
        }
        __builtin_amdgcn_fence(__ATOMIC_RELEASE, "wavefront");
        __builtin_amdgcn_wave_barrier();
        __builtin_amdgcn_fence(__ATOMIC_ACQUIRE, "wavefront");
        const bool coarsen = variance_says_coarsen(m, sv, lane);
        __builtin_amdgcn_wave_barrier();
        if (coarsen) {
          int uval = -1;
          if (lane == 0) {
            u64 key;
            pack_key(mki3(ent.x, ent.y, ent.z), key);
            const int slot = hash_find(t, key);
            const int idx = atomicSub(&t.ctr[CTR_HEAP_COARSE], 1);
            if (idx < 0 || slot < 0) {
              atomicAdd(&t.ctr[CTR_HEAP_COARSE], 1);
              if (slot >= 0) t.keys[slot] = kKeyTomb;
              atomicOr((u32*) &t.ctr[CTR_ERROR], ERR_POOL);
            } else {
              const u32 u = t.heap_coarse[idx];
              t.vals[slot] = u | kValCoarseBit;
              t.desc_coarse[u] = make_int4(ent.x, ent.y, ent.z, 1);
              uval = (int) u;
            }
            const int fi = atomicAdd(&t.ctr[CTR_HEAP_FINE], 1);
            t.heap_fine[fi + 1] = H;
            t.desc_fine[H].w = 0;
          }
          uint4* pz = (uint4*) (t.pool + (size_t) H * kFineBytes);
          const uint4 z = make_uint4(0, 0, 0, 0);
#pragma unroll
          for (int k = 0; k < kFineBytes / 16 / kWave; k++) pz[k * kWave + lane] = z;
          uval = __shfl(uval, 0);
          if (uval >= 0) {
            const int4 ce = make_int4(ent.x, ent.y, ent.z, (int) ((u32) uval | kValCoarseBit));
            const bool collect = coarse_block<false>(c, m, t, f, depth_raw, rgb_raw, ce, lane, 32, trunc_threshold);
            if (FREE && collect) {
              wave_free_coarse(t, ce, lane, deferred);
              if (PROFILE && lane == 0) atomicAdd(&t.prof[PROF_FREED], 1ull);
            }
          }
          continue;
        }
      }
      if (lane == 0) f.summary[H] = make_uint2(__float_as_uint(mn), mx);
    }
    if (FREE && (mn >= trunc_threshold || mx == 0)) {
      if (LZ == 2) wave_zombify(t, f, ent, lane);
      else wave_free_block(t, ent, lane);
      if (PROFILE && lane == 0) atomicAdd(&t.prof[PROF_FREED], 1ull);
    }
    MRH_TS(6);
#ifdef MRH_TRACE
    for (int off = 32; off > 0; off >>= 1) trace_upd += __shfl_xor(trace_upd, off);
    if (lane == 0) { u32 hw; asm volatile("s_getreg_b32 %0, hwreg(HW_REG_HW_ID)" : "=s"(hw)); f.trace[(size_t) e * 8 + 7] = hw | ((u64) trace_upd << 32) | ((u64) ((bb.z * bb.w) & 0x7FFF) << 48) | ((u64) (skip ? 1 : 0) << 63); }
#endif
  }
}

template <bool PROFILE, bool MULTI>
__device__ __forceinline__ void free_range(const Tab& t, const Lists& L, const int n, const int gw, const int nw, const int lane,
                                           u32* __restrict__ deferred) {
  for (int e = gw; e < n; e += nw) {
    if (MULTI) wave_free_any(t, L.cfree[e], lane, deferred);
    else wave_free_block(t, L.cfree[e], lane);
    if (PROFILE && lane == 0) atomicAdd(&t.prof[PROF_FREED], 1ull);
  }
}
template <bool PROFILE, int LZ>
__device__ __forceinline__ void free_candidates(const Tab& t, const Fast& f, const Lists& L, const float trunc_threshold, const int n, const int gw,
                                                const int nw, const int lane, const u32 want_stamp) {
  for (int base = gw * kWave; base < n; base += nw * kWave) {
    const int e = base + lane;
    int4 ent = make_int4(0, 0, 0, 0);
    bool collect = false;
    if (e < n) {
      ent = L.cfree[e];
      const uint2 sm = f.summary[ent.w];
      collect = !(sm.y & kZombieBit) && ((__uint_as_float(sm.x) >= trunc_threshold) || (sm.y == 0u));
      if (sm.y & kZombieBit) {
        u64 key;
        pack_key(mki3(ent.x, ent.y, ent.z), key);
        const int slot = hash_find(t, key);
        if (!(slot >= 0 && f.want[slot] == want_stamp)) atomicAdd(&t.ctr[CTR_ZSKIP], 1);
      }
    }
    u64 todo = __ballot(collect);
    if (PROFILE && todo && lane == 0) atomicAdd(&t.prof[PROF_FREED], (u64) __popcll(todo));
    while (todo) {
      const int src = __ffsll((long long) todo) - 1;
      todo &= todo - 1;
      const int4 b = make_int4(__shfl(ent.x, src), __shfl(ent.y, src), __shfl(ent.z, src), __shfl(ent.w, src));
      if (LZ == 2) wave_zombify(t, f, b, lane);
      else wave_free_block(t, b, lane);
    }
  }
}

__device__ __forceinline__ void frame_epilogue(const Tab& t, const int zero_set, const int n_integrated, const int n_culled, const int lane, const int seq) {
  if (lane < 4) t.ctr[CTR_SET0 + 4 * zero_set + lane] = 0;
  if (lane == 0 && t.h_levels) {
    t.h_levels[0] = t.ctr[CTR_HEAP_FINE];
    t.h_levels[1] = t.ctr[CTR_ZOMBIES];
    t.h_levels[2] = seq;
  }
  if (lane == 0) {
    t.ctr[CTR_COMPACT] = n_integrated;
    t.ctr[CTR_CULLED] = n_culled;
    t.ctr[CTR_FREED_EARLY] = 0;
  }
}

template <bool FREE, bool PROFILE, bool MULTI, bool SAFEDIV, int LZ = 0, bool SPH = false>
__device__ __forceinline__ void back_role(const Cam& c, const Map& m, const Tab& t, const Fast& f, const Lists& L, const int set, const int zero_set,
                                          const float trunc_threshold, const float* __restrict__ depth_raw, const uint8_t* __restrict__ rgb_raw,
                                          u32* __restrict__ deferred, const int gw, const int nw, const int lane, uint2* tile, const u32 want_stamp = 0,
                                          const int seq = 0) {
  const int cs = CTR_SET0 + 4 * set;
  const int nvis = t.ctr[cs + 0];
  const int ncfree = FREE ? t.ctr[cs + 2] : 0;
  const int nkept = t.ctr[cs + 1];
  if (gw == 0) frame_epilogue(t, zero_set, nvis, nkept + t.ctr[cs + 2], lane, seq);
  back_range<FREE, PROFILE, MULTI, SAFEDIV, LZ, SPH>(c, m, t, f, L, trunc_threshold, nvis, gw, nw, lane, tile, depth_raw, rgb_raw, deferred, want_stamp);
  if (FREE) {
    if (LZ) free_candidates<PROFILE, LZ>(t, f, L, trunc_threshold, ncfree, gw, nw, lane, want_stamp);
    else free_range<PROFILE, MULTI>(t, L, ncfree, gw, nw, lane, deferred);
  }
}

template <bool FREE, bool PROFILE, bool MULTI, bool SAFEDIV, int LZ = 0, bool SPH = false>
__global__ __launch_bounds__(256) void k_back(const Cam c, const Map m, const Tab t, const Fast f, const Lists L, const int set, const int zero_set,
                                              const float trunc_threshold, const float* __restrict__ depth_raw,
                                              const uint8_t* __restrict__ rgb_raw, u32* __restrict__ deferred, const u32 want_stamp, const int seq) {
  extern __shared__ __attribute__((aligned(16))) uint2 s_tile[];
  const int wpw = blockDim.x >> 6;
  back_role<FREE, PROFILE, MULTI, SAFEDIV, LZ, SPH>(c, m, t, f, L, set, zero_set, trunc_threshold, depth_raw, rgb_raw, deferred, blockIdx.x * wpw + (threadIdx.x >> 6),
                                               gridDim.x * wpw, threadIdx.x & 63, &s_tile[(threadIdx.x >> 6) * kTileMaxPx], want_stamp, seq);
}

__global__ __launch_bounds__(256) void k_reclaim(const Tab t, const Fast f) {
  const int n = t.ctr[CTR_ZOMBIES];
  const bool by_flag = (u32) n > f.zlist_cap;
  const int total = by_flag ? t.ctr[CTR_HWM_FINE] : n;
  for (int e = blockIdx.x * 256 + threadIdx.x; e < total; e += gridDim.x * 256) {
    int4 ent;
    if (by_flag) {
      ent = t.desc_fine[e];
      if (!(ent.w & 1)) continue;
      ent.w = e;
    } else {
      ent = f.zlist[e];
    }
    const u32 H = (u32) ent.w;
    const u32 old = atomicAnd(&f.summary[H].y, ~kZombieBit);
    if (!(old & kZombieBit)) continue;
    u64 key;
    pack_key(mki3(ent.x, ent.y, ent.z), key);
    hash_erase(t, key);
    const int idx = atomicAdd(&t.ctr[CTR_HEAP_FINE], 1);
    t.heap_fine[idx + 1] = H;
    t.desc_fine[H].w = 0;
  }
}
__global__ void k_reclaim_done(const Tab t) { t.ctr[CTR_ZOMBIES] = 0; }

__global__ __launch_bounds__(256) void k_mr_tail(const Tab t, const u32* __restrict__ deferred, const int low_blocks_to_allocate,
                                                 int* __restrict__ refill_flag) {
  const int n = t.ctr[CTR_NREINT];
  __shared__ int s_base;
  if (threadIdx.x == 0) s_base = n ? atomicAdd(&t.ctr[CTR_HEAP_COARSE], n) : t.ctr[CTR_HEAP_COARSE];
  __syncthreads();
  for (int i = threadIdx.x; i < n; i += 256) t.heap_coarse[s_base + 1 + i] = deferred[i];
  if (threadIdx.x == 0) {
    t.ctr[CTR_NREINT] = 0;
    *refill_flag = (s_base + n + 1 < low_blocks_to_allocate) ? 1 : 0;
  }
}

__global__ __launch_bounds__(256) void k_summarize_visible(const Tab t, const Fast f) {
  const int n = t.ctr[CTR_COMPACT];
  const int lane = threadIdx.x & 63;
  const int gw = blockIdx.x * 4 + (threadIdx.x >> 6), nw = gridDim.x * 4;
  for (int e = gw; e < n; e += nw) {
    const u32 H = (u32) t.compact[e].w;
    const VoxPtr vp = vox_ptr(t, H);
    u32 mnb = 0x7F7FFFFFu, mx = 0;
    for (int v = lane; v < 512; v += 64) {
      const u32 wk = vp.rgbw[v] >> 24;
      mnb = umin_(mnb, wk != 0 ? (__float_as_uint(vp.sdf[v]) & 0x7FFFFFFFu) : 0xFFFFFFFFu);
      mx = umax_(mx, wk);
    }
    mnb = wave_min_u32(mnb);
    mx = wave_max_u32(mx);
    if (lane == 0) f.summary[H] = make_uint2(mnb, mx);
  }
}

__global__ __launch_bounds__(256) void k_summarize_all(const Tab t, const Fast f) {
  const int hwm = t.ctr[CTR_HWM_FINE];
  const int lane = threadIdx.x & 63;
  const int gw = blockIdx.x * 4 + (threadIdx.x >> 6), nw = gridDim.x * 4;
  for (int i = gw; i < (t.multi_res ? 9 : 1) * hwm; i += nw) {
    const bool coarse = i >= hwm;
    const u32 idx = coarse ? (u32) (i - hwm) : (u32) i;
    const int4 d = coarse ? t.desc_coarse[idx] : t.desc_fine[idx];
    if (!(d.w & 1)) continue;
    const VoxPtr vp = vox_ptr(t, coarse ? (idx | kValCoarseBit) : idx);
    u32 mnb = 0x7F7FFFFFu, mx = 0;
    for (int v = lane; v < (coarse ? kCoarseVoxels : 512); v += 64) {
      const u32 wk = vp.rgbw[v] >> 24;
      mnb = umin_(mnb, wk != 0 ? (__float_as_uint(vp.sdf[v]) & 0x7FFFFFFFu) : 0xFFFFFFFFu);
      mx = umax_(mx, wk);
    }
    mnb = wave_min_u32(mnb);
    mx = wave_max_u32(mx);
    if (lane == 0) (coarse ? f.summary_c : f.summary)[idx] = make_uint2(mnb, mx);
  }
}

struct StarveKeys {
  u32 pix[4];
  u32 dep[4];
  u32 mask;
};
template <bool SPH>
__device__ __forceinline__ StarveKeys starve_keys4(const Cam& c, const Map& m, const int4 ent, const int q) {
  const Proj4 P = SPH ? project4_sph(c, m, ent, q) : project4(c, m, ent, q);
  StarveKeys k;
  k.mask = P.mask;
#pragma unroll
  for (int i = 0; i < 4; i++) {
    k.pix[i] = ((P.mask >> i) & 1u) ? (u32) (__mul24(P.row[i], c.cols) + P.col[i]) : 0u;
    k.dep[i] = __float_as_uint(P.pcz[i]);
  }
  return k;
}
template <int PASS, bool SPH>
__global__ __launch_bounds__(256) void k_starve_z(const Cam c, const Map m, const Tab t, const Fast f, const int4* __restrict__ vis, const int set,
                                                  u64* __restrict__ zbuf0, u64* __restrict__ zbuf1) {
  const int count = t.ctr[CTR_SET0 + 4 * set];
  const int lane = threadIdx.x & 63;
  const int gw = blockIdx.x * 4 + (threadIdx.x >> 6), nw = gridDim.x * 4;
  for (int e = __builtin_amdgcn_readfirstlane(gw); e < count; e += nw) {
    const int4 ent = vis[e];
    if (f.summary[ent.w].y & kZombieBit) continue;
    u64 key;
    pack_key(mki3(ent.x, ent.y, ent.z), key);
    const u32 key_hi = (u32) (key >> 31);
    const u64 key_lo = (key & 0x7FFFFFFFull) << 9;
#pragma unroll
    for (int b = 0; b < 2; b++) {
      const int q = lane + 64 * b;
      const StarveKeys k = starve_keys4<SPH>(c, m, ent, q);
#pragma unroll
      for (int i = 0; i < 4; i++) {
        if (!((k.mask >> i) & 1u)) continue;
        const u64 hi = ((u64) k.dep[i] << 32) | key_hi;
        if (PASS == 0) {
          if (zbuf0[k.pix[i]] > hi) atomicMin(&zbuf0[k.pix[i]], hi);
        } else if (zbuf0[k.pix[i]] == hi) {
          const u64 lo = key_lo | (u64) (q * 4 + i);
          if (zbuf1[k.pix[i]] > lo) atomicMin(&zbuf1[k.pix[i]], lo);
        }
      }
    }
  }
}
template <int LZ, bool SPH>
__global__ __launch_bounds__(256) void k_starve_tail(const Cam c, const Map m, const Tab t, const Fast f, const Lists L, const int set,
                                                     const float trunc_threshold, const u32 want_stamp, const u64* __restrict__ zbuf0,
                                                     const u64* __restrict__ zbuf1, u64* __restrict__ clear, const size_t n_clear) {
  const int cs = CTR_SET0 + 4 * set;
  const int nvis = t.ctr[cs + 0], ncfree = t.ctr[cs + 2];
  const int lane = threadIdx.x & 63;
  const int gw = blockIdx.x * 4 + (threadIdx.x >> 6), nw = gridDim.x * 4;
  for (int e = __builtin_amdgcn_readfirstlane(gw); e < nvis; e += nw) {
    const int4 ent = L.vis[e];
    const u32 H = (u32) ent.w;
    if (f.summary[H].y & kZombieBit) continue;
    float4* ps = (float4*) (t.pool + (size_t) H * kFineBytes);
    uint4* pw = (uint4*) (ps + 256);
    u64 key;
    pack_key(mki3(ent.x, ent.y, ent.z), key);
    const u32 key_hi = (u32) (key >> 31);
    const u64 key_lo = (key & 0x7FFFFFFFull) << 9;
    u32 mnb = 0x7F7FFFFFu, mx = 0;
#pragma unroll
    for (int b = 0; b < 2; b++) {
      const int q = lane + 64 * b;
      const float4 S = ps[q];
      uint4 W = pw[q];
      const StarveKeys k = starve_keys4<SPH>(c, m, ent, q);
      u32 w[4] = {W.x, W.y, W.z, W.w};
      u32 won = 0;
#pragma unroll
      for (int i = 0; i < 4; i++) {
        if (!((k.mask >> i) & 1u)) continue;
        const u64 hi = ((u64) k.dep[i] << 32) | key_hi;
        if (zbuf0[k.pix[i]] == hi && zbuf1[k.pix[i]] == (key_lo | (u64) (q * 4 + i))) {
          const u32 wk = w[i] >> 24;
          w[i] = (w[i] & 0x00FFFFFFu) | ((wk > 0 ? wk - 1 : 0) << 24);
          won |= 1u << i;
        }
      }
      if (won) pw[q] = make_uint4(w[0], w[1], w[2], w[3]);
      const float s[4] = {S.x, S.y, S.z, S.w};
#pragma unroll
      for (int i = 0; i < 4; i++) {
        const u32 wk = w[i] >> 24;
        mnb = umin_(mnb, wk != 0 ? (__float_as_uint(s[i]) & 0x7FFFFFFFu) : 0xFFFFFFFFu);
        mx = umax_(mx, wk);
      }
    }
    const u32 mn = wave_min_u32(mnb);
    mx = wave_max_u32(mx);
    if (lane == 0) f.summary[H] = make_uint2(mn, mx);
    if (__uint_as_float(mn) >= trunc_threshold || mx == 0) {
      if (LZ == 2) wave_zombify(t, f, ent, lane);
      else wave_free_block(t, ent, lane);
      if (lane == 0) atomicAdd(&t.prof[PROF_FREED], 1ull);
    }
  }
  if (LZ) free_candidates<true, LZ>(t, f, L, trunc_threshold, ncfree, gw, nw, lane, want_stamp);
  else free_range<true, false>(t, L, ncfree, gw, nw, lane, nullptr);
  for (size_t i = (size_t) blockIdx.x * 256 + threadIdx.x; i < n_clear; i += (size_t) gridDim.x * 256) clear[i] = 0x7FFFFFFFFFFFFFFFull;
}

__global__ __launch_bounds__(256) void k_free_lists(const Tab t, const Fast f, const Lists L, const int set, const float trunc_threshold) {
  const int cs = CTR_SET0 + 4 * set;
  const int nvis = t.ctr[cs + 0], ncfree = t.ctr[cs + 2];
  const int lane = threadIdx.x & 63;
  const int gw = blockIdx.x * 4 + (threadIdx.x >> 6);
  const int nw = gridDim.x * 4;
  for (int e = gw; e < nvis + ncfree; e += nw) {
    const int4 ent = e < nvis ? L.vis[e] : L.cfree[e - nvis];
    bool fr = e >= nvis;
    if (!fr) {
      const uint2 sm = f.summary[ent.w];
      fr = (__uint_as_float(sm.x) >= trunc_threshold) || (sm.y == 0u);
    }
    if (fr) {
      wave_free_block(t, ent, lane);
      if (lane == 0) atomicAdd(&t.prof[PROF_FREED], 1ull);
    }
  }
}

}
```

mrhash_amd/csrc/mrh_frame.h:

```cpp
#pragma once
namespace {

int resync_front(mrh_ctx* c) {
  PipeState& ps = c->ps;
  if (!ps.front_needs_sync) return MRH_OK;
  HIP_TRY(c, hipStreamSynchronize(c->stream));
  ps.front_needs_sync = false;
  ps.base = ps.seq - 1;
  return MRH_OK;
}

FrameInputs read_inputs(const mrh_ctx* c) {
  FrameInputs in;
  in.cam = c->cam;
  in.d_depth = c->d_depth; in.d_rgb = c->d_rgb;
  in.depth_rows = c->depth_rows; in.depth_cols = c->depth_cols; in.rgb_rows = c->rgb_rows; in.rgb_cols = c->rgb_cols;
  const UpRing* rings[2] = {&c->up_depth, &c->up_rgb};
  for (int i = 0; i < 2; i++) in.ring[i] = {rings[i]->cur, rings[i]->last_copy, {rings[i]->waited[0], rings[i]->waited[1]}};
  return in;
}
void apply_inputs(mrh_ctx* c, const FrameInputs& in) {
  c->cam = in.cam;
  c->d_depth = in.d_depth; c->d_rgb = in.d_rgb;
  c->depth_rows = in.depth_rows; c->depth_cols = in.depth_cols; c->rgb_rows = in.rgb_rows; c->rgb_cols = in.rgb_cols;
  UpRing* rings[2] = {&c->up_depth, &c->up_rgb};
  for (int i = 0; i < 2; i++) {
    rings[i]->cur = in.ring[i].cur; rings[i]->last_copy = in.ring[i].last_copy;
    rings[i]->waited[0] = in.ring[i].waited[0]; rings[i]->waited[1] = in.ring[i].waited[1];
  }
}

bool census_due(const mrh_ctx* c) { return c->census_period >= 0 && (c->table_dirty || c->frames_since_census >= (uint64_t) c->census_period); }
int maintain_table(mrh_ctx* c) {
  if (c->pending || !census_due(c)) return MRH_OK;
  hipStream_t s = c->stream;
  const Tab& t = c->tab;
  const int grid = (int) std::min<uint64_t>(2048, (c->slots + 255) / 256);
  main_stream_changed_map(c);
  k_table_census<<<grid, 256, 0, s>>>(t, (size_t) c->slots);
  k_rehash_decide<<<1, 1, 0, s>>>(t, (u32) (c->slots / 4), c->census_force);
  k_rehash_clear<<<grid, 256, 0, s>>>(t, (size_t) c->slots);
  k_rehash_insert<<<1024, 256, 0, s>>>(t);
  c->frames_since_census = 0;
  c->table_dirty = false;
  HIP_TRY(c, hipGetLastError());
  return MRH_OK;
}

int frame_upkeep(mrh_ctx* c) {
  if (census_due(c) && (c->ps.npend > 0 || c->ps.zombies_possible)) {
    const int rc = strict_point(c);
    if (rc) return rc;
  }
  const int rc = maintain_table(c);
  if (rc) return rc;
  c->frames_since_census++;
  return MRH_OK;
}

void refill_coarse(mrh_ctx* c) {
  k_refill_decide<<<1, 64, 0, c->stream>>>(c->tab, c->low_blocks_to_allocate, c->d_flag);
  k_refill<<<(c->low_blocks_to_allocate + 255) / 256, 256, 0, c->stream>>>(c->tab, c->low_blocks_to_allocate, c->d_flag);
}

void plan_begin(const mrh_ctx* c, FramePlan& p, const FrameKind kind, const int n_frames_invalidate) {
  p = FramePlan{};
  p.kind = kind;
  p.max_num_frames = n_frames_invalidate < 0 ? c->p.n_frames_invalidate_voxels : n_frames_invalidate;
  p.starve_now = p.max_num_frames > 0 && c->frames > 0 && c->frames % (uint64_t) p.max_num_frames == 0;
  p.gc_thr = c->map.trunc + c->map.trunc_scale * c->cam.max_depth;
}

void plan_frame(const mrh_ctx* c, FramePlan& p, const int n_frames_invalidate) {
  plan_begin(c, p, FRAME_SERIAL, n_frames_invalidate);
  const Cam& k = c->cam;
  if (c->tab.multi_res) {
    const bool fused = c->mr_fused && !c->profile && p.max_num_frames > 0 && !p.starve_now && !c->mr_next_general && c->frames >= 2 && !c->spherical;
    p.kind = fused ? FRAME_FUSED_MR : FRAME_GENERAL;
  }
  p.starve_fused = c->starve_fused && c->p.shard_count <= 1 && p.kind == FRAME_SERIAL;
  p.starve_in_pipe = p.starve_now && p.starve_fused && !c->starve_serial;
  p.gc_inline = p.kind == FRAME_FUSED_MR || (p.kind == FRAME_SERIAL && p.max_num_frames > 0 && !p.starve_now);
  p.safe_div = c->map.half_vs_two_steps || c->map.wsum_two_steps;
  p.sph = c->spherical;
  p.tiles_x = (k.cols + kRayTile - 1) / kRayTile;
  p.n_tiles = p.tiles_x * ((k.rows + kRayTile - 1) / kRayTile);
}

void take_slots(mrh_ctx* c, FramePlan& p) {
  PipeState& ps = c->ps;
  if (p.kind != FRAME_FUSED_MR) {
    p.seq = (int) (ps.seq & 0x3FFFFFFF);
    p.ring = p.kind == FRAME_PIPELINED ? (int) (ps.seq % kPipeRing) : 0;
    ps.seq++;
  }
  p.set = (int) (ps.fast_frames % kListSets);
  p.zero_set = (p.set + kListSets - 1) % kListSets;
  ps.fast_frames++;
  p.stamp = (u32) ((c->frames + 1) & 0x3FFFFFFFu);
}

int take_event_pair(mrh_ctx* c, EvPair& e) {
  if (!c->ev_pool.empty()) { e = c->ev_pool.back(); c->ev_pool.pop_back(); return MRH_OK; }
  if (c->ev_pending.size() >= 4096) {
    HIP_TRY(c, hipStreamSynchronize(c->stream));
    const int r = drain_events(c);
    if (r) return r;
    e = c->ev_pool.back(); c->ev_pool.pop_back();
    return MRH_OK;
  }
  HIP_TRY(c, event_new(c, e.a, true)); HIP_TRY(c, event_new(c, e.b, true));
  return MRH_OK;
}

Lists ring_lists(const mrh_ctx* c, const int i) {
  if (i == 0) return Lists{c->tab.compact, c->fast.bbox, c->d_cfree, c->d_zmin, (u32) c->num_blocks};
  const PipeState& ps = c->ps;
  return Lists{ps.ring_vis[i], ps.ring_bbox[i], ps.ring_cfree[i], ps.ring_zmin[i], (u32) c->num_blocks};
}

struct BackArgs {
  Cam c; Map m; Tab t; Fast f; Lists L;
  int set, zero_set;
  float thr;
  const float* depth_raw; const uint8_t* rgb_raw; u32* deferred;
  u32 want_stamp; int seq;
};
struct FrontArgs {
  Cam c; Map m; Tab t; Fast f; Lists L;
  const float* depth; const uint8_t* rgb;
  int tiles_x, n_tiles; u32 stamp; int set, gc_on; float thr;
  int n_refill, low_blocks_to_allocate; const int* refill_flag;
};
BackArgs back_args(const mrh_ctx* c, const FramePlan& p, const Cam& k, const Fast& f, const Lists& L) {
  if (p.kind == FRAME_FUSED_MR) return {k, c->map, c->tab, f, L, p.set, p.zero_set, p.gc_thr, c->d_depth, c->d_rgb, (u32*) c->d_reint, 0u, 0};
  return {k, c->map, c->tab, f, L, p.set, p.zero_set, p.gc_thr, nullptr, nullptr, nullptr, p.stamp, p.seq};
}
int refill_wgs(const mrh_ctx* c) { return (c->low_blocks_to_allocate + 255) / 256; }
FrontArgs front_args(const mrh_ctx* c, const FramePlan& p, const Cam& k, const Fast& f, const Lists& L) {
  const int gc_on = p.max_num_frames > 0 ? 1 : 0;
  if (p.kind == FRAME_FUSED_MR)
    return {k, c->map, c->tab, f, L, c->d_depth, c->d_rgb, p.tiles_x, p.n_tiles, p.stamp, p.set, gc_on, p.gc_thr, refill_wgs(c), c->low_blocks_to_allocate, c->d_flag};
  return {k, c->map, c->tab, f, L, c->d_depth, c->d_rgb, p.tiles_x, p.n_tiles, p.stamp, p.set, gc_on, p.gc_thr, 0, 0, nullptr};
}

template <bool FREE, bool PROFILE, bool MULTI, bool SAFEDIV, int LZ, bool SPH>
void back_as(const int grid, hipStream_t s, const EvPair* ev, const BackArgs& a) {
  const size_t lds = (size_t) 4 * kTileMaxPx * sizeof(uint2);
  if (ev) hipExtLaunchKernelGGL((k_back<FREE, PROFILE, MULTI, SAFEDIV, LZ, SPH>), dim3(grid), dim3(256), (uint32_t) lds, s, ev->a, ev->b, 0u,
                                a.c, a.m, a.t, a.f, a.L, a.set, a.zero_set, a.thr, a.depth_raw, a.rgb_raw, a.deferred, a.want_stamp, a.seq);
  else k_back<FREE, PROFILE, MULTI, SAFEDIV, LZ, SPH><<<grid, 256, lds, s>>>(a.c, a.m, a.t, a.f, a.L, a.set, a.zero_set, a.thr, a.depth_raw, a.rgb_raw,
                                                                             a.deferred, a.want_stamp, a.seq);
}
template <bool FREE, bool PROFILE, int LZ>
void back_single_res(const bool safe_div, const bool sph, const int grid, hipStream_t s, const EvPair* ev, const BackArgs& a) {
  if (safe_div && sph) back_as<FREE, PROFILE, false, true, LZ, true>(grid, s, ev, a);
  else if (safe_div) back_as<FREE, PROFILE, false, true, LZ, false>(grid, s, ev, a);
  else if (sph) back_as<FREE, PROFILE, false, false, LZ, true>(grid, s, ev, a);
  else back_as<FREE, PROFILE, false, false, LZ, false>(grid, s, ev, a);
}
void launch_back(const FramePlan& p, const int grid, hipStream_t s, const EvPair* ev, const BackArgs& a) {
  if (p.kind == FRAME_FUSED_MR) {
    if (p.safe_div) back_as<true, false, true, true, 0, false>(grid, s, ev, a);
    else back_as<true, false, true, false, 0, false>(grid, s, ev, a);
  } else if (p.kind == FRAME_PIPELINED) {
    if (p.gc_inline && ev) back_single_res<true, true, 2>(p.safe_div, p.sph, grid, s, ev, a);
    else if (p.gc_inline) back_single_res<true, false, 2>(p.safe_div, p.sph, grid, s, ev, a);
    else back_single_res<false, false, 2>(p.safe_div, p.sph, grid, s, ev, a);
  } else {
    if (p.gc_inline && ev) back_single_res<true, true, 0>(p.safe_div, p.sph, grid, s, ev, a);
    else if (p.gc_inline) back_single_res<true, false, 0>(p.safe_div, p.sph, grid, s, ev, a);
    else back_single_res<false, false, 0>(p.safe_div, p.sph, grid, s, ev, a);
  }
}

template <bool PROFILE, bool MULTI, bool LAZY, bool SPH>
void front_as(const int grid, hipStream_t s, const EvPair* ev, const FrontArgs& a) {
  if (ev) hipExtLaunchKernelGGL((k_front<PROFILE, MULTI, LAZY, SPH>), dim3(grid), dim3(256), 0, s, ev->a, ev->b, 0u, a.c, a.m, a.t, a.f, a.L, a.depth, a.rgb,
                                a.tiles_x, a.n_tiles, a.stamp, a.set, a.gc_on, a.thr, a.n_refill, a.low_blocks_to_allocate, a.refill_flag);
  else k_front<PROFILE, MULTI, LAZY, SPH><<<grid, 256, 0, s>>>(a.c, a.m, a.t, a.f, a.L, a.depth, a.rgb, a.tiles_x, a.n_tiles, a.stamp, a.set, a.gc_on, a.thr,
                                                               a.n_refill, a.low_blocks_to_allocate, a.refill_flag);
}
template <bool PROFILE>
void front_single_res(const bool lazy, const bool sph, const int grid, hipStream_t s, const EvPair* ev, const FrontArgs& a) {
  if (lazy && sph) front_as<PROFILE, false, true, true>(grid, s, ev, a);
  else if (lazy) front_as<PROFILE, false, true, false>(grid, s, ev, a);
  else if (sph) front_as<PROFILE, false, false, true>(grid, s, ev, a);
  else front_as<PROFILE, false, false, false>(grid, s, ev, a);
}
void launch_front(const FramePlan& p, const int grid, hipStream_t s, const EvPair* ev, const FrontArgs& a) {
  if (p.kind == FRAME_FUSED_MR) front_as<false, true, false, false>(grid, s, nullptr, a);
  else if (ev) front_single_res<true>(p.kind == FRAME_PIPELINED, p.sph, grid, s, ev, a);
  else front_single_res<false>(p.kind == FRAME_PIPELINED, p.sph, grid, s, nullptr, a);
}

int ensure_zbuf(mrh_ctx* c, size_t npix) { return regrow(c, c->d_zbuf, c->zbuf_n, npix, 2 * npix * sizeof(u64)); }

int ensure_zfused(mrh_ctx* c, const size_t npix) {
  PipeState& ps = c->ps;
  if (ps.zfused_n >= npix) return MRH_OK;
  ps.zfused_clean[0] = ps.zfused_clean[1] = false;
  return regrow(c, ps.d_zfused, ps.zfused_n, npix, 4 * npix * sizeof(u64));
}

template <bool SPH, int LZ>
void starve_fused_as(hipStream_t s, const Cam& k, const Map& m, const Tab& t, const Fast& f, const Lists& L, const FramePlan& p, u64* z0, u64* z1, u64* other,
                     const size_t npix) {
  const int grid = 2048;
  k_starve_z<0, SPH><<<grid, 256, 0, s>>>(k, m, t, f, L.vis, p.set, z0, z1);
  k_starve_z<1, SPH><<<grid, 256, 0, s>>>(k, m, t, f, L.vis, p.set, z0, z1);
  k_starve_tail<LZ, SPH><<<grid, 256, 0, s>>>(k, m, t, f, L, p.set, p.gc_thr, p.stamp, z0, z1, other, 2 * npix);
}
int launch_starve_fused(mrh_ctx* c, const FramePlan& p, const Cam& k, const Fast& f, const Lists& L) {
  PipeState& ps = c->ps;
  const size_t npix = (size_t) k.rows * k.cols;
  hipStream_t s = c->stream;
  const int rc = ensure_zfused(c, npix);
  if (rc) return rc;
  if (ps.zfused_clean_npix != npix) ps.zfused_clean[0] = ps.zfused_clean[1] = false;
  ps.zfused_clean_npix = npix;
  const int pair = ps.zfused_next, q = pair ^ 1;
  u64* z0 = ps.d_zfused + (size_t) pair * 2 * ps.zfused_n;
  u64* z1 = z0 + npix;
  u64* other = ps.d_zfused + (size_t) q * 2 * ps.zfused_n;
  if (!ps.zfused_clean[pair]) k_fill_u64<<<256, 256, 0, s>>>(z0, 2 * npix, 0x7FFFFFFFFFFFFFFFull);
  ps.zfused_clean[pair] = false;
  const bool lazy = p.kind == FRAME_PIPELINED;
  if (k.model && lazy) starve_fused_as<true, 2>(s, k, c->map, c->tab, f, L, p, z0, z1, other, npix);
  else if (k.model) starve_fused_as<true, 0>(s, k, c->map, c->tab, f, L, p, z0, z1, other, npix);
  else if (lazy) starve_fused_as<false, 2>(s, k, c->map, c->tab, f, L, p, z0, z1, other, npix);
  else starve_fused_as<false, 0>(s, k, c->map, c->tab, f, L, p, z0, z1, other, npix);
  HIP_TRY(c, hipGetLastError());
  ps.zfused_clean[q] = true;
  ps.zfused_next = q;
  c->n_starve_fused++;
  return MRH_OK;
}

int launch_starve(mrh_ctx* c, int pass) {
  const Cam& k = c->cam;
  const size_t npix = (size_t) k.rows * k.cols;
  hipStream_t s = c->stream;
  if (pass == 0) {
    int rc = ensure_zbuf(c, npix);
    if (rc) return rc;
    k_fill_u64<<<256, 256, 0, s>>>(c->d_zbuf, 2 * npix, 0x7FFFFFFFFFFFFFFFull);
    k_starve<0><<<c->integrate_grid, 512, 0, s>>>(k, c->map, c->tab, c->d_zbuf, c->d_zbuf + npix);
  } else if (pass == 1) {
    k_starve<1><<<c->integrate_grid, 512, 0, s>>>(k, c->map, c->tab, c->d_zbuf, c->d_zbuf + npix);
  } else {
    k_starve<2><<<c->integrate_grid, 512, 0, s>>>(k, c->map, c->tab, c->d_zbuf, c->d_zbuf + npix);
  }
  return MRH_OK;
}

int frame_tail(mrh_ctx* c, const FramePlan& p) {
  hipStream_t s = c->stream;
  const Tab& t = c->tab;
  if (p.kind == FRAME_GENERAL) {
    if (p.max_num_frames > 0) {
      k_gc_identify<<<c->integrate_grid, 512, 0, s>>>(t, p.gc_thr, c->d_decision);
      if (c->profile) k_gc_free<true><<<256, 256, 0, s>>>(t, c->d_decision);
      else k_gc_free<false><<<256, 256, 0, s>>>(t, c->d_decision);
    }
    if (!t.multi_res) c->fast_summaries_stale = true;
  } else if (!t.multi_res) {
    if (p.starve_now) k_summarize_visible<<<1024, 256, 0, s>>>(t, c->fast);
    if (p.max_num_frames > 0 && !p.gc_inline) k_free_lists<<<256, 256, 0, s>>>(t, c->fast, ring_lists(c, 0), p.set, p.gc_thr);
  }
  c->frames++;
  HIP_TRY(c, hipGetLastError());
  return MRH_OK;
}

int starve_and_tail(mrh_ctx* c, const FramePlan& p) {
  if (p.starve_now) {
    int rc = launch_starve(c, 0);
    if (rc) return rc;
    if (c->p.shard_count > 1 && c->comm) {
      const size_t npix = (size_t) c->cam.rows * c->cam.cols;
      rc = comm_allreduce_zbuf(c, c->d_zbuf, npix);
      if (rc) return rc;
      if ((rc = launch_starve(c, 1))) return rc;
      rc = comm_allreduce_zbuf(c, c->d_zbuf + npix, npix);
      if (rc) return rc;
      if ((rc = launch_starve(c, 2))) return rc;
      return frame_tail(c, p);
    }
    if (c->p.shard_count > 1) {
      HIP_TRY(c, hipStreamSynchronize(c->stream));
      c->pending = 1;
      return MRH_PENDING_EXCHANGE;
    }
    if ((rc = launch_starve(c, 1))) return rc;
    if ((rc = launch_starve(c, 2))) return rc;
  }
  return frame_tail(c, p);
}

int resume_frame(mrh_ctx* c) {
  if (c->pending == 1) {
    launch_starve(c, 1);
    HIP_TRY(c, hipStreamSynchronize(c->stream));
    c->pending = 2;
    return MRH_PENDING_EXCHANGE;
  }
  if (c->pending == 2) {
    launch_starve(c, 2);
    c->pending = 0;
    const int rc = frame_tail(c, c->plan);
    if (rc < 0) return rc;
    const int mrc = mark_frame(c);
    return mrc ? mrc : rc;
  }
  return fail(c, MRH_ERR_STATE, "mrh_integrate_resume: no exchange is pending");
}

int launch_pending(mrh_ctx* c, const bool count_skips = false) {
  PipeState& ps = c->ps;
  if (!ps.npend) return MRH_OK;
  const PendingBack pb = ps.pendq[0];
  for (int i = 1; i < ps.npend; i++) ps.pendq[i - 1] = ps.pendq[i];
  ps.npend--;
  const FramePlan& p = pb.plan;
  hipStream_t s = c->stream;
  const hipError_t q = c->pipe_always_wait ? hipErrorNotReady : hipEventQuery(ps.ev_front[p.ring]);
  if (q == hipErrorNotReady) {
    (void) hipGetLastError();
    HIP_TRY(c, hipStreamWaitEvent(s, ps.ev_front[p.ring], 0));
    c->dbg_waits++;
  } else if (q != hipSuccess) {
    return fail(c, MRH_ERR_DEVICE, "mrh_integrate: front half of a pipelined frame: %s", hipGetErrorString(q));
  }
  const bool profiled = pb.ev.a != nullptr;
  if (count_skips) HIP_TRY(c, hipMemsetAsync(&c->tab.ctr[CTR_ZSKIP], 0, sizeof(int), s));
  if (profiled)
    k_count_updates<<<c->fused_grid, 256, 0, s>>>(pb.cam, c->map, c->tab, pb.f, c->d_cnt_partials, CTR_SET0 + 4 * p.set, pb.L.vis, pb.L.cfree, p.stamp,
                                                  pb.count_zombies ? 1 : 0);
  launch_back(p, c->pipe_grid, s, profiled ? &pb.ev : nullptr, back_args(c, p, pb.cam, pb.f, pb.L));
  if (profiled) c->ev_pending.push_back(pb.ev);
  if (p.gc_inline) ps.zombies_possible = true;
  if (p.starve_now) {
    const int src = launch_starve_fused(c, p, pb.cam, pb.f, pb.L);
    if (src) return src;
    ps.zombies_possible = true;
  }
  HIP_TRY(c, hipGetLastError());
  return pb.report_seq && c->peek_enabled ? post_report(c, pb.report_seq, s) : MRH_OK;
}

int strict_point(mrh_ctx* c) {
  PipeState& ps = c->ps;
  while (ps.npend) {
    const int rc = launch_pending(c, ps.npend == 1);
    if (rc) return rc;
  }
  if (!ps.zombies_possible) return MRH_OK;
  main_stream_changed_map(c);
  k_reclaim<<<64, 256, 0, c->stream>>>(c->tab, c->fast);
  k_reclaim_done<<<1, 1, 0, c->stream>>>(c->tab);
  if (c->peek_enabled && c->frame_seq > 1) {
    const uint64_t seq = c->frame_seq - 1;
    if (c->peek_seq[seq % 8] == seq && c->peek_done[seq % 8]) {
      if (const int rc = post_report(c, seq, c->stream)) return rc;
    }
  }
  ps.zombies_possible = false;
  ps.lazy_run = 0;
  HIP_TRY(c, hipGetLastError());
  return MRH_OK;
}

int ensure_pipe_state(mrh_ctx* c) {
  PipeState& ps = c->ps;
  if (ps.stream_front) return MRH_OK;
  const size_t cap = c->num_blocks;
  for (hipEvent_t& e : ps.ev_front) if (!e) HIP_TRY(c, event_new(c, e, false));
  for (int i = 1; i < kPipeRing; i++) {
    if (!ps.ring_vis[i]) HIP_TRY(c, dev_alloc(c, ps.ring_vis[i], cap * sizeof(int4)));
    if (!ps.ring_bbox[i]) HIP_TRY(c, dev_alloc(c, ps.ring_bbox[i], cap * sizeof(int4)));
    if (!ps.ring_cfree[i]) HIP_TRY(c, dev_alloc(c, ps.ring_cfree[i], cap * sizeof(int4)));
    if (!ps.ring_zmin[i]) HIP_TRY(c, dev_alloc(c, ps.ring_zmin[i], cap * sizeof(float)));
  }
  if (!c->fast.zlist) HIP_TRY(c, dev_alloc(c, c->fast.zlist, cap * sizeof(int4)));
  if (!ps.want_ring) HIP_TRY(c, dev_alloc(c, ps.want_ring, (size_t) kPipeRing * c->slots * sizeof(u32)));
  main_stream_changed_map(c);
  HIP_TRY(c, hipMemsetAsync(ps.want_ring, 0, (size_t) kPipeRing * c->slots * sizeof(u32), c->stream));
  if (!ps.h_levels) HIP_TRY(c, pinned_alloc(c, ps.h_levels, 4 * sizeof(int)));
  HIP_TRY(c, hipStreamCreateWithFlags(&ps.stream_front, hipStreamNonBlocking));
  ps.h_levels[0] = (int) c->num_blocks - 1; ps.h_levels[1] = 0; ps.h_levels[2] = -1;
  c->tab.h_levels = ps.h_levels;
  return MRH_OK;
}

int ensure_frame_dcx(mrh_ctx* c, const size_t npix) {
  PipeState& ps = c->ps;
  if (ps.npix >= npix) return MRH_OK;
  {
    const int rc = strict_point(c);
    if (rc) return rc;
  }
  if (ps.stream_front) HIP_TRY(c, hipStreamSynchronize(ps.stream_front));
  HIP_TRY(c, hipStreamSynchronize(c->stream));
  for (uint2*& d : ps.dcx) HIP_TRY(c, dev_free(c, d));
  ps.npix = 0;
  const int n = ps.stream_front ? kPipeRing : 1;
  for (int i = 0; i < n; i++) HIP_TRY(c, dev_alloc(c, ps.dcx[i], npix * sizeof(uint2)));
  ps.npix = npix;
  return MRH_OK;
}

bool pool_roomy(const mrh_ctx* c) {
  const volatile int* lev = c->ps.h_levels;
  const int64_t free_known = (int64_t) lev[0] + 1, zombies_known = lev[1];
  return free_known >= (int64_t) (c->num_blocks / 4) && zombies_known <= (int64_t) (c->num_blocks / 8);
}

int wait_for_ring_slot(mrh_ctx* c, const FramePlan& p) {
  const int64_t need = (int64_t) p.seq - kPipeRing + 2;
  if (need <= (int64_t) c->ps.base) return MRH_OK;
  const auto t0 = std::chrono::steady_clock::now();
  while ((int64_t) ((volatile int*) c->ps.h_levels)[2] < need) {
    MRH_CPU_RELAX();
    if (std::chrono::steady_clock::now() - t0 > std::chrono::seconds(10)) return fail(c, MRH_ERR_DEVICE, "mrh_integrate: the integration of frame %lld never started", (long long) need);
  }
  c->dbg_spin_us += std::chrono::duration<double, std::micro>(std::chrono::steady_clock::now() - t0).count();
  return MRH_OK;
}

bool frame_may_pipeline(const mrh_ctx* c, const FramePlan& p) {
  const bool resident_inputs = c->up_depth.cur < 0 && c->up_rgb.cur < 0;
  return c->pipe && (!p.starve_now || p.starve_in_pipe) && pool_roomy(c) && c->ps.lazy_run < c->pipe_period && c->ps.sync_streak < 3 &&
         (resident_inputs || c->pipe_uploads);
}
int integrate_single_res_frame(mrh_ctx* c, FramePlan& p) {
  PipeState& ps = c->ps;
  int rc = MRH_OK;
  hipStream_t s = c->stream;
  const Cam& k = c->cam;
  if (c->pipe) {
    rc = ensure_pipe_state(c);
    if (rc) return rc;
  }
  rc = ensure_frame_dcx(c, (size_t) k.rows * k.cols);
  if (rc) return rc;
  if (c->fast_summaries_stale) {
    rc = strict_point(c);
    if (rc) return rc;
    main_stream_changed_map(c);
    k_summarize_all<<<2048, 256, 0, s>>>(c->tab, c->fast);
    c->fast_summaries_stale = false;
  }
  ps.sync_streak = ps.flushed_since_frame ? ps.sync_streak + 1 : 0;
  ps.flushed_since_frame = false;
  const bool lazy = frame_may_pipeline(c, p);
  if (lazy) p.kind = FRAME_PIPELINED;
  else if ((rc = strict_point(c))) return rc;
  rc = send_uploads(c, lazy ? ps.stream_front : s);
  if (rc) return rc;
  take_slots(c, p);
  c->fast.dcx = ps.dcx[p.ring];
  c->fast.want = ps.want_ring + (size_t) p.ring * c->slots;
  const Fast f = c->fast;
  const Lists L = ring_lists(c, p.ring);
  EvPair ev = {nullptr, nullptr}, evf = {nullptr, nullptr};
  if (c->profile) {
    rc = take_event_pair(c, evf);
    if (rc) return rc;
    rc = take_event_pair(c, ev);
    if (rc) return rc;
  }
  const FrontArgs front = front_args(c, p, k, f, L);
  ps.last_frame_lazy = lazy;
  if (lazy) {
    rc = resync_front(c);
    if (rc) return rc;
    rc = wait_for_ring_slot(c, p);
    if (rc) return rc;
    c->dbg_lazy_frames++;
    const auto t_api = std::chrono::steady_clock::now();
    launch_front(p, p.n_tiles + c->sweep_wgs, ps.stream_front, c->profile ? &evf : nullptr, front);
    HIP_TRY(c, hipEventRecord(ps.ev_front[p.ring], ps.stream_front));
    if (c->profile) c->ev_pending_front.push_back(evf);
    const bool zombies_before = ps.zombies_possible;
    while (ps.npend >= c->pipe_defer) {
      rc = launch_pending(c);
      if (rc) return rc;
    }
    PendingBack& pb = ps.pendq[ps.npend++];
    pb.plan = p; pb.cam = k; pb.f = f; pb.L = L;
    pb.ev = ev;
    pb.report_seq = 0;
    pb.count_zombies = zombies_before || ps.zombies_possible || p.gc_inline;
    ps.lazy_run++;
    c->frames++;
    c->dbg_api_us += std::chrono::duration<double, std::micro>(std::chrono::steady_clock::now() - t_api).count();
    HIP_TRY(c, hipGetLastError());
    return MRH_OK;
  }
  main_stream_changed_map(c);
  launch_front(p, p.n_tiles + c->sweep_wgs, s, c->profile ? &evf : nullptr, front);
  if (c->profile) {
    c->ev_pending_front.push_back(evf);
    k_count_updates<<<c->fused_grid, 256, 0, s>>>(k, c->map, c->tab, f, c->d_cnt_partials, CTR_SET0 + 4 * p.set, L.vis, L.cfree, p.stamp, 0);
  }
  launch_back(p, c->fused_grid, s, c->profile ? &ev : nullptr, back_args(c, p, k, f, L));
  if (c->profile) c->ev_pending.push_back(ev);
  if (p.starve_now && p.starve_fused) {
    rc = launch_starve_fused(c, p, k, f, L);
    if (rc) return rc;
    c->frames++;
    return MRH_OK;
  }
  return starve_and_tail(c, p);
}

int integrate_fused_mr_frame(mrh_ctx* c, FramePlan& p) {
  hipStream_t s = c->stream;
  const Cam& k = c->cam;
  const Tab& t = c->tab;
  int rc = ensure_frame_dcx(c, (size_t) k.rows * k.cols);
  if (rc) return rc;
  c->fast.dcx = c->ps.dcx[0];
  const Fast& f = c->fast;
  take_slots(c, p);
  const Lists L = ring_lists(c, 0);
  if (!c->mr_summaries_valid) {
    k_summarize_all<<<2048, 256, 0, s>>>(t, f);
    c->mr_summaries_valid = true;
  }
  if (!c->refill_flag_valid) k_refill_decide<<<1, 64, 0, s>>>(t, c->low_blocks_to_allocate, c->d_flag);
  launch_front(p, p.n_tiles + c->sweep_wgs_mr + refill_wgs(c), s, nullptr, front_args(c, p, k, f, L));
  launch_back(p, c->fused_grid, s, nullptr, back_args(c, p, k, f, L));
  k_mr_tail<<<1, 256, 0, s>>>(t, (const u32*) c->d_reint, c->low_blocks_to_allocate, c->d_flag);
  rc = starve_and_tail(c, p);
  c->refill_flag_valid = rc == MRH_OK;
  return rc;
}

int integrate_general_frame(mrh_ctx* c, const FramePlan& p) {
  hipStream_t s = c->stream;
  const Cam& k = c->cam;
  const Map& m = c->map;
  const Tab& t = c->tab;
  refill_coarse(c);
  const float* depth_img = c->d_depth;
  if (c->spherical) {
    const size_t npix = (size_t) k.rows * k.cols;
    const int rc = regrow(c, c->d_cloud, c->cloud_n, npix, npix * sizeof(float));
    if (rc) return rc;
    k_cloud_depth<<<(int) ((npix + 255) / 256), 256, 0, s>>>(k, c->d_depth, c->d_cloud);
    depth_img = c->d_cloud;
  }
  const dim3 tiles((k.cols + kTile - 1) / kTile, (k.rows + kTile - 1) / kTile);
  if (c->profile) k_alloc<true><<<tiles, dim3(kTile, kTile), 0, s>>>(k, m, t, depth_img);
  else k_alloc<false><<<tiles, dim3(kTile, kTile), 0, s>>>(k, m, t, depth_img);
  k_compact<<<512, 256, 0, s>>>(k, m, t, 1);

  if (c->profile) {
    EvPair ev;
    const int rc = take_event_pair(c, ev);
    if (rc) return rc;
    HIP_TRY(c, hipEventRecord(ev.a, s));
    k_integrate<true><<<c->integrate_grid, 512, 0, s>>>(k, m, t, depth_img, c->d_rgb, c->d_upd_partials);
    HIP_TRY(c, hipEventRecord(ev.b, s));
    c->ev_pending.push_back(ev);
  } else {
    k_integrate<false><<<c->integrate_grid, 512, 0, s>>>(k, m, t, depth_img, c->d_rgb, c->d_upd_partials);
  }

  if (c->frames > 0) {
    HIP_TRY(c, hipMemsetAsync(&t.ctr[CTR_NREALLOC], 0, 2 * sizeof(int), s));
    k_check_var<<<2048, 64, 0, s>>>(m, t, c->d_realloc);
    k_realloc<<<64, 256, 0, s>>>(t, c->d_realloc, c->d_reint);
    k_compact<<<512, 256, 0, s>>>(k, m, t, 1);
    k_reintegrate<<<1024, 64, 0, s>>>(k, m, t, depth_img, c->d_rgb, c->d_reint);
  }

  return starve_and_tail(c, p);
}

int integrate_checks(mrh_ctx* c) {
  if (c->pending) return fail(c, MRH_ERR_STATE, "mrh_integrate: an exchange is pending (call mrh_integrate_resume)");
  if (c->halo_upper) return fail(c, MRH_ERR_STATE, "mrh_integrate: halo blocks of other shards are present (call mrh_drop_blocks(MRH_DROP_HALO) after the extraction)");
  if (!c->has_camera) return fail(c, MRH_ERR_STATE, "mrh_integrate: set_camera has not been called");
  if (c->comm && c->p.shard_count > 1) {
    int cr = 0, cw = 1;
    if (!comm_matches_sharding(c, &cr, &cw) && !getenv("MRH_COMM_ALLOW_SHARD_MISMATCH"))
      return fail(c, MRH_ERR_STATE, "mrh_integrate: the context is shard %d of %d, the attached communicator rank %d of %d", c->p.shard_rank, c->p.shard_count, cr, cw);
  }
  if (!c->d_depth || !c->d_rgb) return fail(c, MRH_ERR_STATE, "mrh_integrate: depth and rgb images are required");
  const Cam& k = c->cam;
  if (c->depth_rows != k.rows || c->depth_cols != k.cols || c->rgb_rows != k.rows || c->rgb_cols != k.cols)
    return fail(c, MRH_ERR_INVALID_ARG, "mrh_integrate: image shape does not match the camera");
  return MRH_OK;
}

int integrate_frame(mrh_ctx* c, const int n_frames_invalidate) {
  int rc = integrate_checks(c);
  if (rc) return rc;
  rc = frame_upkeep(c);
  if (rc) return rc;
  FramePlan& p = c->plan;
  plan_frame(c, p, n_frames_invalidate);
  if (p.kind == FRAME_GENERAL) {
    c->mr_summaries_valid = false;
    c->mr_next_general = p.starve_now || c->frames == 0;
    c->refill_flag_valid = false;
  }
  const size_t npix = (size_t) c->cam.rows * c->cam.cols;
  if (p.max_num_frames > 0 && p.starve_fused && c->ps.zfused_n < npix) {
    rc = ensure_zfused(c, npix);
    if (rc) return rc;
    k_fill_u64<<<512, 256, 0, c->stream>>>(c->ps.d_zfused, 4 * npix, 0x7FFFFFFFFFFFFFFFull);
    c->ps.zfused_clean[0] = c->ps.zfused_clean[1] = true;
    c->ps.zfused_clean_npix = npix;
  }
  if (p.kind == FRAME_SERIAL) return integrate_single_res_frame(c, p);
  rc = send_uploads(c, c->stream);
  if (rc) return rc;
  return p.kind == FRAME_FUSED_MR ? integrate_fused_mr_frame(c, p) : integrate_general_frame(c, p);
}

int run_frame(mrh_ctx* c, const int n_frames_invalidate) {
  const int rc = integrate_frame(c, n_frames_invalidate);
  if (rc < 0) return rc;
  const int mrc = mark_frame(c);
  return mrc ? mrc : rc;
}

bool frame_is_deferrable(const mrh_ctx* c) {
  const bool up_d = c->up_depth.cur >= 0 && c->d_depth == c->up_depth.s[c->up_depth.cur].d && !c->up_depth.waited[0] && !c->up_depth.waited[1];
  const bool up_c = c->up_rgb.cur >= 0 && c->d_rgb == c->up_rgb.s[c->up_rgb.cur].d && !c->up_rgb.waited[0] && !c->up_rgb.waited[1];
  return c->defer_uploads && (up_d || up_c) && c->p.shard_count <= 1 && !c->comm && !c->profile;
}
int defer_frame(mrh_ctx* c, const int n_frames_invalidate) {
  const int rc = integrate_checks(c);
  if (rc) return rc;
  c->deferred = {true, n_frames_invalidate, read_inputs(c)};
  return MRH_OK;
}
int flush_deferred(mrh_ctx* c) {
  DeferredFrame& d = c->deferred;
  if (!d.on) return MRH_OK;
  d.on = false;
  FrameInputs now = read_inputs(c);
  apply_inputs(c, d.in);
  const int rc = run_frame(c, d.n_inval);
  const UpRing* rings[2] = {&c->up_depth, &c->up_rgb};
  for (int i = 0; i < 2; i++)
    if (now.ring[i].last_copy == d.in.ring[i].last_copy) { now.ring[i].waited[0] = rings[i]->waited[0]; now.ring[i].waited[1] = rings[i]->waited[1]; }
  apply_inputs(c, now);
  return rc;
}

}
```

Before: 27440 frames/s.

## Split kernel args into hot fields and a device-resident cold struct

Kernel arguments for the front and back kernels are reduced to a small set of hot pointers. Rarely used table and fast-path fields move into a device-resident Cold struct, published once at init and read through the constant address space only on slow paths. The LDS tile changes from interleaved uint2 to two planar u32 arrays padded by one element, the free path is skipped when a wave has no candidates, and the summary reduction is rewritten to save an op. The aim is to shrink the kernarg footprint and SGPR pressure and to reduce LDS bank conflicts, at the cost of extra indirection on cold paths and a sync point whenever the cold struct is republished.

```diff
diff --git a/mrhash_amd/csrc/mrh_context.h b/mrhash_amd/csrc/mrh_context.h
--- a/mrhash_amd/csrc/mrh_context.h
+++ b/mrhash_amd/csrc/mrh_context.h
@@ -207,6 +207,7 @@
   u32* d_misc = nullptr;
   float* d_rcp_w = nullptr;
   Fast fast;
+  Cold* d_cold = nullptr;
   int pipe = 1;
   int pipe_grid = 1024;
   int pipe_uploads = 0;
@@ -468,6 +469,21 @@
   ps.front_needs_sync = false;
 }
 
+int publish_cold(mrh_ctx* c) {
+  const int rc = strict_point(c);
+  if (rc) return rc;
+  if (c->ps.stream_front) HIP_TRY(c, hipStreamSynchronize(c->ps.stream_front));
+  HIP_TRY(c, hipStreamSynchronize(c->stream));
+  main_stream_changed_map(c);
+  if (!c->d_cold) HIP_TRY(c, dev_alloc(c, c->d_cold, sizeof(Cold)));
+  Cold h;
+  h.t = c->tab;
+  h.f = c->fast;
+  h.f.dcx = nullptr; h.f.want = nullptr;
+  HIP_TRY(c, hipMemcpy(c->d_cold, &h, sizeof h, hipMemcpyHostToDevice));
+  return MRH_OK;
+}
+
 int init_buffers(mrh_ctx* c) {
   hipStream_t s = c->stream;
   c->mr_next_general = true;
@@ -505,7 +521,7 @@
   c->n_front_ms = 0;
   c->tris.clear(); c->V.clear(); c->C.clear(); c->F.clear();
   c->last_triangles = 0;
-  return MRH_OK;
+  return publish_cold(c);
 }
 
 int create_checks(const mrh_params* p) {
diff --git a/mrhash_amd/csrc/mrh_fast.h b/mrhash_amd/csrc/mrh_fast.h
--- a/mrhash_amd/csrc/mrh_fast.h
+++ b/mrhash_amd/csrc/mrh_fast.h
@@ -8,6 +8,7 @@
 constexpr int CTR_FREED_EARLY = 13;
 constexpr float kFltMax = 3.402823466e+38f;
 constexpr int kTileMaxPx = 576;
+constexpr int kTilePlane = kTileMaxPx + 1;
 
 struct Fast {
   uint2* dcx;
@@ -28,13 +29,63 @@
   asm volatile("s_waitcnt lgkmcnt(0)\n\ts_memrealtime %0\n\ts_waitcnt lgkmcnt(0)" : "=s"(t) : : "memory");
   return t;
 }
-#define MRH_TS(slot) do { if (lane == 0) f.trace[(size_t) e * 8 + (slot)] = trace_now(); } while (0)
+#define MRH_TS(slot) do { if (lane == 0) h.trace[(size_t) e * 8 + (slot)] = trace_now(); } while (0)
 constexpr size_t kTraceFront = 32768;
-#define MRH_TSF(slot) do { if (threadIdx.x == 0) f.trace[(kTraceFront + blockIdx.x) * 8 + (slot)] = trace_now(); } while (0)
+#define MRH_TSF(slot) do { if (threadIdx.x == 0) h.trace[(kTraceFront + blockIdx.x) * 8 + (slot)] = trace_now(); } while (0)
 #else
 #define MRH_TS(slot) do { } while (0)
 #define MRH_TSF(slot) do { } while (0)
 #endif
+
+struct Cold {
+  Tab t;
+  Fast f;
+};
+#define MRH_CONST_AS __attribute__((address_space(4)))
+typedef const MRH_CONST_AS Cold* ColdRef;
+__device__ __forceinline__ Tab cold_tab(const Cold* cold) {
+  const ColdRef q = (ColdRef) cold;
+  Tab t;
+  t.keys = q->t.keys; t.vals = q->t.vals; t.slot_mask = q->t.slot_mask; t.max_probe = q->t.max_probe;
+  t.heap_fine = q->t.heap_fine; t.heap_coarse = q->t.heap_coarse; t.desc_fine = q->t.desc_fine; t.desc_coarse = q->t.desc_coarse;
+  t.pool = q->t.pool; t.compact = q->t.compact; t.ctr = q->t.ctr; t.prof = q->t.prof;
+  t.cap_blocks = q->t.cap_blocks; t.multi_res = q->t.multi_res; t.h_levels = q->t.h_levels;
+  return t;
+}
+__device__ __forceinline__ Fast cold_fast(const Cold* cold, uint2* dcx, u32* want) {
+  const ColdRef q = (ColdRef) cold;
+  Fast f;
+  f.dcx = dcx; f.want = want;
+  f.summary = q->f.summary; f.zlist_cap = q->f.zlist_cap; f.bbox = q->f.bbox; f.summary_c = q->f.summary_c; f.zlist = q->f.zlist;
+#ifdef MRH_TRACE
+  f.trace = q->f.trace;
+#endif
+  return f;
+}
+__device__ __forceinline__ u64* cold_prof(const Cold* cold) { return ((ColdRef) cold)->t.prof; }
+
+struct BackHot {
+  char* pool;
+  int* ctr;
+  uint2* dcx;
+  uint2* summary;
+  u32* want;
+  const Cold* cold;
+#ifdef MRH_TRACE
+  u64* trace;
+#endif
+};
+struct FrontHot {
+  u64* keys;
+  u32 slot_mask, max_probe;
+  int* ctr;
+  uint2* dcx;
+  u32* want;
+  const Cold* cold;
+#ifdef MRH_TRACE
+  u64* trace;
+#endif
+};
 
 __device__ __forceinline__ void wave_free_block(const Tab& t, const int4 ent, const int lane) {
   const u32 H = (u32) ent.w;
@@ -201,7 +252,7 @@
   u32 cv[4];
 };
 __device__ __forceinline__ float tile_inv_w(const int4 bb) { return __builtin_amdgcn_rcpf((float) bb.z); }
-__device__ __forceinline__ void tile_issue(const Cam& c, const Fast& f, const int4 bb, const int lane, TileRegs& tr) {
+__device__ __forceinline__ void tile_issue(const Cam& c, const uint2* __restrict__ dcx, const int4 bb, const int lane, TileRegs& tr) {
   const int npx = bb.z * bb.w;
   if (npx <= 0) return;
   const float inv_w = tile_inv_w(bb);
@@ -211,12 +262,12 @@
     const int r = (int) (((float) p + 0.5f) * inv_w);
     const int cc = p - r * bb.z;
     const u32 g = (u32) (__mul24(bb.y + r, c.cols) + bb.x + cc);
-    const uint2 v = f.dcx[g];
+    const uint2 v = dcx[g];
     tr.dv[j] = __uint_as_float(v.x);
     tr.cv[j] = v.y;
   }
 }
-__device__ __forceinline__ float tile_commit(const Cam& c, const Map& m, const Fast& f, const int4 bb, const int lane, uint2* tile,
+__device__ __forceinline__ float tile_commit(const Cam& c, const Map& m, const uint2* __restrict__ dcx, const int4 bb, const int lane, u32* tile,
                                              const TileRegs& tr) {
   const int npx = bb.z * bb.w;
   float reach = 0.f;
@@ -224,7 +275,7 @@
 #pragma unroll
   for (int j = 0; j < 4; j++) {
     const int p = lane + 64 * j;
-    if (p < npx) tile[p] = make_uint2(__float_as_uint(tr.dv[j]), tr.cv[j]);
+    if (p < npx) { tile[p] = __float_as_uint(tr.dv[j]); tile[kTilePlane + p] = tr.cv[j]; }
     reach = __uint_as_float(umax_(__float_as_uint(reach), __float_as_uint(pixel_reach(c, m, tr.dv[j]))));
   }
   if (npx > 256) {
@@ -239,14 +290,14 @@
         const int r = (int) (((float) p + 0.5f) * inv_w);
         const int cc = p - r * bb.z;
         const u32 g = (u32) (__mul24(bb.y + r, c.cols) + bb.x + cc);
-        const uint2 v = f.dcx[g];
+        const uint2 v = dcx[g];
         dv[j] = __uint_as_float(v.x);
         cv[j] = v.y;
       }
 #pragma unroll
       for (int j = 0; j < 2; j++) {
         const int p = p0 + 64 * j;
-        if (p < npx) tile[p] = make_uint2(__float_as_uint(dv[j]), cv[j]);
+        if (p < npx) { tile[p] = __float_as_uint(dv[j]); tile[kTilePlane + p] = cv[j]; }
         reach = __uint_as_float(umax_(__float_as_uint(reach), __float_as_uint(pixel_reach(c, m, dv[j]))));
       }
     }
@@ -255,7 +306,7 @@
 }
 
 template <int NB>
-__device__ __forceinline__ void tile_lookup(const Fast& f, const int cols, const int4 bb, const uint2* tile, const Proj4 (&P)[NB],
+__device__ __forceinline__ void tile_lookup(const uint2* __restrict__ dcx, const int cols, const int4 bb, const u32* tile, const Proj4 (&P)[NB],
                                             const bool (&ok)[NB][4], float (&d)[NB][4], u32 (&cpx)[NB][4]) {
   bool miss[NB][4], any_miss = false;
   u32 li[NB][4];
@@ -273,9 +324,8 @@
   for (int b = 0; b < NB; b++)
 #pragma unroll
     for (int k = 0; k < 4; k++) {
-      const uint2 px = tile[li[b][k]];
-      d[b][k] = __uint_as_float(px.x);
-      cpx[b][k] = px.y;
+      d[b][k] = __uint_as_float(tile[li[b][k]]);
+      cpx[b][k] = tile[kTilePlane + li[b][k]];
     }
   if (__ballot(any_miss)) {
 #pragma unroll
@@ -284,7 +334,7 @@
       for (int k = 0; k < 4; k++)
         if (miss[b][k]) {
           const u32 pix = (u32) (__mul24(P[b].row[k], cols) + P[b].col[k]);
-          const uint2 v = f.dcx[pix];
+          const uint2 v = dcx[pix];
           d[b][k] = __uint_as_float(v.x);
           cpx[b][k] = v.y;
         }
diff --git a/mrhash_amd/csrc/mrh_fast2.h b/mrhash_amd/csrc/mrh_fast2.h
--- a/mrhash_amd/csrc/mrh_fast2.h
+++ b/mrhash_amd/csrc/mrh_fast2.h
@@ -17,6 +17,12 @@
 };
 
 __device__ __forceinline__ int desc_w(u32 stamp) { return (int) (1u | (stamp << 1)); }
+
+__device__ __forceinline__ Tab probe_tab(const FrontHot& h) {
+  Tab t = {};
+  t.keys = h.keys; t.slot_mask = h.slot_mask; t.max_probe = h.max_probe;
+  return t;
+}
 
 struct FrontShared {
   u64 set[kRayCap];
@@ -105,8 +111,9 @@
 }
 
 template <bool MARK, bool SPH = false>
-__device__ __forceinline__ u32 wave_insert_keys(const Cam& c, const Map& m, const Tab& t, const Fast& f, const Lists& L, const u64 key,
+__device__ __forceinline__ u32 wave_insert_keys(const Cam& c, const Map& m, const FrontHot& h, const Lists& L, const u64 key,
                                                 const u32 stamp, const int cs, const int hwm0) {
+  const Tab tp = probe_tab(h);
   const bool active = key != kKeyEmpty;
   const i3 b = active ? unpack_key(key) : mki3(0, 0, 0);
   bool won = false;
@@ -114,18 +121,21 @@
   int claim;
   u64 claim_val;
   if (active) {
-    const int found = hash_find_claim(t, key, claim, claim_val);
+    const int found = hash_find_claim(tp, key, claim, claim_val);
     if (found >= 0) {
-      if (MARK) f.want[found] = stamp;
+      if (MARK) h.want[found] = stamp;
     } else if (SPH ? block_in_frustum_approx_m(c, m.vs, b) : block_in_frustum_approx(c, m.vs, b)) {
-      slot = hash_insert_at(t, key, claim, claim_val);
-      if (slot == -2) atomicOr((u32*) &t.ctr[CTR_ERROR], ERR_TABLE);
+      slot = hash_insert_at(tp, key, claim, claim_val);
+      if (slot == -2) atomicOr((u32*) &h.ctr[CTR_ERROR], ERR_TABLE);
       won = slot >= 0;
     }
   }
   const u64 ballot = __ballot(won);
   u32 inserted = 0;
   if (ballot) {
+    Tab t = cold_tab(h.cold);
+    t.ctr = h.ctr;
+    const Fast f = cold_fast(h.cold, h.dcx, h.want);
     const int leader = __ffsll((long long) ballot) - 1;
     int hb = 0;
     if ((int) lane_id() == leader) hb = atomicSub(&t.ctr[CTR_HEAP_FINE], __popcll(ballot));
@@ -151,26 +161,26 @@
 }
 
 template <bool PROFILE, bool MARK, bool SPH = false>
-__device__ __forceinline__ void front_tile(const Cam& c, const Map& m, const Tab& t, const Fast& f, const Lists& L,
+__device__ __forceinline__ void front_tile(const Cam& c, const Map& m, const FrontHot& h, const Lists& L,
                                            const float* __restrict__ depth, const uint8_t* __restrict__ rgb, const int tiles_x,
                                            const int tile_id, const u32 stamp, const int cs, FrontShared& sh) {
   constexpr int NT = 256;
   const int tid = threadIdx.x;
-  const int hwm0 = t.ctr[CTR_HWM_FINE];
+  const int hwm0 = h.ctr[CTR_HWM_FINE];
   MRH_TSF(1);
   float d;
-  const bool slow = tile_rays<SPH>(c, m, f.dcx, depth, rgb, tiles_x, tile_id, sh, d);
+  const bool slow = tile_rays<SPH>(c, m, h.dcx, depth, rgb, tiles_x, tile_id, sh, d);
   MRH_TSF(3);
   if (slow) {
     const int ty = tile_id / tiles_x, tx = tile_id - ty * tiles_x;
-    tile_slow_pixel<PROFILE, MARK, SPH>(c, m, t, f, L, ty * kRayTile + (tid >> 4), tx * kRayTile + (tid & 15), d, stamp, cs, hwm0);
+    tile_slow_pixel<PROFILE, MARK, SPH>(c, m, cold_tab(h.cold), cold_fast(h.cold, h.dcx, h.want), L, ty * kRayTile + (tid >> 4), tx * kRayTile + (tid & 15), d, stamp, cs, hwm0);
   }
   const int n = (int) sh.count;
   u32 my_inserted = 0;
 #pragma unroll 1
   for (int base = 0; base < n; base += NT) {
     const int i = base + tid;
-    my_inserted += wave_insert_keys<MARK, SPH>(c, m, t, f, L, i < n ? sh.list[i] : kKeyEmpty, stamp, cs, hwm0);
+    my_inserted += wave_insert_keys<MARK, SPH>(c, m, h, L, i < n ? sh.list[i] : kKeyEmpty, stamp, cs, hwm0);
   }
   MRH_TSF(4);
 #ifdef MRH_TRACE
@@ -179,24 +189,27 @@
     asm volatile("s_getreg_b32 %0, hwreg(HW_REG_HW_ID)" : "=s"(hw));
     u32 xcc;
     asm volatile("s_getreg_b32 %0, hwreg(HW_REG_XCC_ID)" : "=s"(xcc));
-    f.trace[(kTraceFront + blockIdx.x) * 8 + 7] = (u64) n;
-    f.trace[(kTraceFront + blockIdx.x) * 8 + 5] = (u64) hw | ((u64) xcc << 32);
+    h.trace[(kTraceFront + blockIdx.x) * 8 + 7] = (u64) n;
+    h.trace[(kTraceFront + blockIdx.x) * 8 + 5] = (u64) hw | ((u64) xcc << 32);
   }
 #endif
   if (PROFILE) {
     if (my_inserted) atomicAdd(&sh.inserted, my_inserted);
     __syncthreads();
-    if (tid == 0 && sh.inserted) atomicAdd(&t.prof[PROF_INSERTED], (u64) sh.inserted);
+    if (tid == 0 && sh.inserted) atomicAdd(&cold_prof(h.cold)[PROF_INSERTED], (u64) sh.inserted);
   }
 }
 
 template <bool MULTI, bool DEFER = false, bool SPH = false>
-__device__ __forceinline__ void front_sweep(const Cam& c, const Map& m, const Tab& t, const Fast& f, const Lists& L, const u32 stamp,
+__device__ __forceinline__ void front_sweep(const Cam& c, const Map& m, const FrontHot& h, const Lists& L, const u32 stamp,
                                             const int cs, const int gc_on, const float trunc_threshold, const int sw, const int n_sweep,
                                             FrontShared& sh) {
   constexpr int NT = 256;
   const int tid = threadIdx.x;
-  const int hwm = t.ctr[CTR_HWM_FINE];
+  const int hwm = h.ctr[CTR_HWM_FINE];
+  Tab t = cold_tab(h.cold);
+  t.ctr = h.ctr;
+  const Fast f = cold_fast(h.cold, h.dcx, h.want);
   int4* st_vis = (int4*) sh.list;
   int4* st_free = (int4*) sh.set;
   constexpr int kStVis = kRayCap * 8 / 32, kStFree = kRayCap * 8 / 16;
@@ -296,7 +309,7 @@
   if (tid == 0 && sh.nkeep) atomicAdd(&t.ctr[cs + 1], sh.nkeep);
   MRH_TSF(4);
 #ifdef MRH_TRACE
-  if (tid == 0) f.trace[(kTraceFront + blockIdx.x) * 8 + 7] = (u64) (hwm / n_sweep) | (1ull << 63);
+  if (tid == 0) h.trace[(kTraceFront + blockIdx.x) * 8 + 7] = (u64) (hwm / n_sweep) | (1ull << 63);
 #endif
 }
 
@@ -313,7 +326,7 @@
 }
 
 template <bool PROFILE, bool MULTI, bool LAZY = false, bool SPH = false>
-__global__ __launch_bounds__(256) void k_front(const Cam c, const Map m, const Tab t, const Fast f, const Lists L,
+__global__ __launch_bounds__(256) void k_front(const Cam c, const Map m, const FrontHot h, const Lists L,
                                                const float* __restrict__ depth, const uint8_t* __restrict__ rgb, const int tiles_x,
                                                const int n_tiles, const u32 stamp, const int set, const int gc_on,
                                                const float trunc_threshold, const int n_refill, const int low_blocks_to_allocate,
@@ -322,9 +335,9 @@
   const int cs = CTR_SET0 + 4 * set;
   const int n_sweep = (int) gridDim.x - n_tiles - n_refill;
   MRH_TSF(0);
-  if (MULTI && (int) blockIdx.x >= n_sweep + n_tiles) front_refill(t, low_blocks_to_allocate, refill_flag, (int) blockIdx.x - n_sweep - n_tiles);
-  else if ((int) blockIdx.x >= n_sweep) front_tile<PROFILE, LAZY, SPH>(c, m, t, f, L, depth, rgb, tiles_x, (int) blockIdx.x - n_sweep, stamp, cs, sh);
-  else front_sweep<MULTI, LAZY, SPH>(c, m, t, f, L, stamp, cs, gc_on, trunc_threshold, (int) blockIdx.x, n_sweep, sh);
+  if (MULTI && (int) blockIdx.x >= n_sweep + n_tiles) front_refill(cold_tab(h.cold), low_blocks_to_allocate, refill_flag, (int) blockIdx.x - n_sweep - n_tiles);
+  else if ((int) blockIdx.x >= n_sweep) front_tile<PROFILE, LAZY, SPH>(c, m, h, L, depth, rgb, tiles_x, (int) blockIdx.x - n_sweep, stamp, cs, sh);
+  else front_sweep<MULTI, LAZY, SPH>(c, m, h, L, stamp, cs, gc_on, trunc_threshold, (int) blockIdx.x, n_sweep, sh);
 }
 
 __device__ __forceinline__ int4 wave_bbox(const Cam& c, const float vs, const int4 ent, const int lane, float& zmin_out) {
@@ -399,9 +412,8 @@
     const i3 pi = mki3(ent.x * kBlockSide + 2 * (v & 3), ent.y * kBlockSide + 2 * ((v >> 2) & 3), ent.z * kBlockSide + 2 * (v >> 4));
     if (integrate_voxel<VARIANCE>(c, m, depth, rgb, pi, &sd, &sq, &rw)) { vp.sdf[v] = sd; vp.sumsq[v] = sq; vp.rgbw[v] = rw; }
   }
-  const u32 wk = rw >> 24;
-  const float mn = __uint_as_float(wave_min_u32(umin_(0x7F7FFFFFu, wk != 0 ? (__float_as_uint(sd) & 0x7FFFFFFFu) : 0xFFFFFFFFu)));
-  const u32 mx = wave_max_u32(wk);
+  const float mn = __uint_as_float(wave_min_u32(umin_(0x7F7FFFFFu, rw > 0x00FFFFFFu ? (__float_as_uint(sd) & 0x7FFFFFFFu) : 0xFFFFFFFFu)));
+  const u32 mx = wave_max_u32(rw) >> 24;
   if (lane == 0) f.summary_c[u] = make_uint2(__float_as_uint(mn), mx);
   return mn >= trunc_threshold || mx == 0;
 }
@@ -444,24 +456,30 @@
 #pragma unroll
   for (int k = 0; k < kFineBytes / 16 / kWave; k++) p[k * kWave + lane] = z;
 }
-__device__ __forceinline__ bool zombie_wanted(const Tab& t, const Fast& f, const int4 ent, const u32 want_stamp, const int lane) {
+__device__ __forceinline__ bool zombie_wanted(const Tab& t, const u32* __restrict__ want, const int4 ent, const u32 want_stamp, const int lane) {
   int wanted = 0;
   if (lane == 0) {
     u64 key;
     pack_key(mki3(ent.x, ent.y, ent.z), key);
     const int slot = hash_find(t, key);
-    wanted = (slot >= 0 && f.want[slot] == want_stamp) ? 1 : 0;
+    wanted = (slot >= 0 && want[slot] == want_stamp) ? 1 : 0;
   }
   return __builtin_amdgcn_readfirstlane(wanted) != 0;
 }
 
 template <bool FREE, bool PROFILE, bool MULTI, bool SAFEDIV, int LZ = 0, bool SPH = false>
-__device__ __forceinline__ void back_range(const Cam& c, const Map& m, const Tab& t, const Fast& f, const Lists& L,
+__device__ __forceinline__ void back_range(const Cam& c, const Map& m, const BackHot& h, const Lists& L,
                                            const float trunc_threshold, const int n, const int gw, const int nw, const int lane,
                                            uint2* tile, const float* __restrict__ depth_raw, const uint8_t* __restrict__ rgb_raw,
                                            u32* __restrict__ deferred, const u32 want_stamp = 0) {
   static_assert(!(MULTI && LZ), "multi-resolution maps are not pipelined");
   static_assert(!(MULTI && SPH), "multi-resolution maps under the spherical model take the general kernels");
+  Tab tm = {};
+  Fast fm = {};
+  if (MULTI) { tm = cold_tab(h.cold); tm.pool = h.pool; tm.ctr = h.ctr; fm = cold_fast(h.cold, h.dcx, h.want); fm.summary = h.summary; }
+  const Tab& t = tm;
+  const Fast& f = fm;
+  u32* const tile_px = (u32*) tile;
   for (int e = __builtin_amdgcn_readfirstlane(gw); e < n; e += nw) {
     MRH_TS(0);
     int4 ent, bb;
@@ -476,11 +494,11 @@
       continue;
     }
     const u32 H = (u32) ent.w;
-    float4* ps = (float4*) (t.pool + (size_t) H * kFineBytes);
+    float4* ps = (float4*) (h.pool + (size_t) H * kFineBytes);
     float4* pq = ps + 128;
     uint4* pw = (uint4*) (ps + 256);
     uint2 sm0 = make_uint2(0u, 0u);
-    if (LZ) sm0 = f.summary[H];
+    if (LZ) sm0 = h.summary[H];
     float4 S[2];
     uint4 W[2];
 #pragma unroll
@@ -496,19 +514,20 @@
     u32 cpx[2][4];
     MRH_TS(1);
     TileRegs tr;
-    tile_issue(c, f, bb, lane, tr);
+    tile_issue(c, h.dcx, bb, lane, tr);
 #pragma unroll
     for (int b = 0; b < 2; b++) P[b] = SPH ? project4_sph(c, m, ent, lane + 64 * b) : project4(c, m, ent, lane + 64 * b);
     if (LZ && (sm0.y & kZombieBit)) {
-      if (!zombie_wanted(t, f, ent, want_stamp, lane)) {
-        if (lane == 0) atomicAdd(&t.ctr[CTR_ZSKIP], 1);
+      const Tab tc = cold_tab(h.cold);
+      if (!zombie_wanted(tc, h.want, ent, want_stamp, lane)) {
+        if (lane == 0) atomicAdd(&tc.ctr[CTR_ZSKIP], 1);
         continue;
       }
       sm0 = make_uint2(0x7F7FFFFFu, 0u);
-      if (lane == 0) f.summary[H] = sm0;
-      if (PROFILE && lane == 0) atomicAdd(&t.prof[PROF_INSERTED], 1ull);
-    }
-    const float reach = tile_commit(c, m, f, bb, lane, tile, tr);
+      if (lane == 0) h.summary[H] = sm0;
+      if (PROFILE && lane == 0) atomicAdd(&cold_prof(h.cold)[PROF_INSERTED], 1ull);
+    }
+    const float reach = tile_commit(c, m, h.dcx, bb, lane, tile_px, tr);
     const bool skip = bb.z != 0 && __ballot(!(reach + 1e-4f <= zmin)) == 0;
     float mn;
     u32 mx;
@@ -516,7 +535,7 @@
     u32 trace_upd = 0;
 #endif
     if (skip) {
-      const uint2 sm = LZ ? sm0 : f.summary[H];
+      const uint2 sm = LZ ? sm0 : h.summary[H];
       mn = __uint_as_float(sm.x);
       mx = sm.y;
     } else {
@@ -530,11 +549,11 @@
       for (int b = 0; b < 2; b++)
 #pragma unroll
         for (int k = 0; k < 4; k++) ok[b][k] = proj_ok<SPH>(c, P[b], k);
-      tile_lookup<2>(f, c.cols, bb, tile, P, ok, d, cpx);
+      tile_lookup<2>(h.dcx, c.cols, bb, tile_px, P, ok, d, cpx);
       __builtin_amdgcn_wave_barrier();
       MRH_TS(4);
       u32 mnb = 0x7F7FFFFFu;
-      mx = 0;
+      u32 mxw = 0;
 #pragma unroll
       for (int b = 0; b < 2; b++) {
         const int q = lane + 64 * b;
@@ -568,14 +587,13 @@
         }
 #pragma unroll
         for (int k = 0; k < 4; k++) {
-          const u32 wk = w[k] >> 24;
           const u32 ab = __float_as_uint(s[k]) & 0x7FFFFFFFu;
-          mnb = umin_(mnb, wk != 0 ? ab : 0xFFFFFFFFu);
-          mx = umax_(mx, wk);
+          mnb = umin_(mnb, w[k] > 0x00FFFFFFu ? ab : 0xFFFFFFFFu);
+          mxw = umax_(mxw, w[k]);
         }
       }
       mn = __uint_as_float(wave_min_u32(mnb));
-      mx = wave_max_u32(mx);
+      mx = wave_max_u32(mxw) >> 24;
       MRH_TS(5);
       if (MULTI) {
         __builtin_amdgcn_wave_barrier();
@@ -614,7 +632,7 @@
             t.heap_fine[fi + 1] = H;
             t.desc_fine[H].w = 0;
           }
-          uint4* pz = (uint4*) (t.pool + (size_t) H * kFineBytes);
+          uint4* pz = (uint4*) (h.pool + (size_t) H * kFineBytes);
           const uint4 z = make_uint4(0, 0, 0, 0);
 #pragma unroll
           for (int k = 0; k < kFineBytes / 16 / kWave; k++) pz[k * kWave + lane] = z;
@@ -630,17 +648,23 @@
           continue;
         }
       }
-      if (lane == 0) f.summary[H] = make_uint2(__float_as_uint(mn), mx);
+      if (lane == 0) h.summary[H] = make_uint2(__float_as_uint(mn), mx);
     }
     if (FREE && (mn >= trunc_threshold || mx == 0)) {
-      if (LZ == 2) wave_zombify(t, f, ent, lane);
-      else wave_free_block(t, ent, lane);
-      if (PROFILE && lane == 0) atomicAdd(&t.prof[PROF_FREED], 1ull);
+      const Tab tc = cold_tab(h.cold);
+      if (LZ == 2) {
+        Fast fc = cold_fast(h.cold, h.dcx, h.want);
+        fc.summary = h.summary;
+        wave_zombify(tc, fc, ent, lane);
+      } else {
+        wave_free_block(tc, ent, lane);
+      }
+      if (PROFILE && lane == 0) atomicAdd(&tc.prof[PROF_FREED], 1ull);
     }
     MRH_TS(6);
 #ifdef MRH_TRACE
     for (int off = 32; off > 0; off >>= 1) trace_upd += __shfl_xor(trace_upd, off);
-    if (lane == 0) { u32 hw; asm volatile("s_getreg_b32 %0, hwreg(HW_REG_HW_ID)" : "=s"(hw)); f.trace[(size_t) e * 8 + 7] = hw | ((u64) trace_upd << 32) | ((u64) ((bb.z * bb.w) & 0x7FFF) << 48) | ((u64) (skip ? 1 : 0) << 63); }
+    if (lane == 0) { u32 hw; asm volatile("s_getreg_b32 %0, hwreg(HW_REG_HW_ID)" : "=s"(hw)); h.trace[(size_t) e * 8 + 7] = hw | ((u64) trace_upd << 32) | ((u64) ((bb.z * bb.w) & 0x7FFF) << 48) | ((u64) (skip ? 1 : 0) << 63); }
 #endif
   }
 }
@@ -684,45 +708,48 @@
   }
 }
 
-__device__ __forceinline__ void frame_epilogue(const Tab& t, const int zero_set, const int n_integrated, const int n_culled, const int lane, const int seq) {
-  if (lane < 4) t.ctr[CTR_SET0 + 4 * zero_set + lane] = 0;
-  if (lane == 0 && t.h_levels) {
-    t.h_levels[0] = t.ctr[CTR_HEAP_FINE];
-    t.h_levels[1] = t.ctr[CTR_ZOMBIES];
-    t.h_levels[2] = seq;
+__device__ __forceinline__ void frame_epilogue(int* __restrict__ ctr, int* __restrict__ h_levels, const int zero_set, const int n_integrated, const int n_culled,
+                                               const int lane, const int seq) {
+  if (lane < 4) ctr[CTR_SET0 + 4 * zero_set + lane] = 0;
+  if (lane == 0 && h_levels) {
+    h_levels[0] = ctr[CTR_HEAP_FINE];
+    h_levels[1] = ctr[CTR_ZOMBIES];
+    h_levels[2] = seq;
   }
   if (lane == 0) {
-    t.ctr[CTR_COMPACT] = n_integrated;
-    t.ctr[CTR_CULLED] = n_culled;
-    t.ctr[CTR_FREED_EARLY] = 0;
+    ctr[CTR_COMPACT] = n_integrated;
+    ctr[CTR_CULLED] = n_culled;
+    ctr[CTR_FREED_EARLY] = 0;
   }
 }
 
 template <bool FREE, bool PROFILE, bool MULTI, bool SAFEDIV, int LZ = 0, bool SPH = false>
-__device__ __forceinline__ void back_role(const Cam& c, const Map& m, const Tab& t, const Fast& f, const Lists& L, const int set, const int zero_set,
+__device__ __forceinline__ void back_role(const Cam& c, const Map& m, const BackHot& h, const Lists& L, const int set, const int zero_set,
                                           const float trunc_threshold, const float* __restrict__ depth_raw, const uint8_t* __restrict__ rgb_raw,
                                           u32* __restrict__ deferred, const int gw, const int nw, const int lane, uint2* tile, const u32 want_stamp = 0,
                                           const int seq = 0) {
   const int cs = CTR_SET0 + 4 * set;
-  const int nvis = t.ctr[cs + 0];
-  const int ncfree = FREE ? t.ctr[cs + 2] : 0;
-  const int nkept = t.ctr[cs + 1];
-  if (gw == 0) frame_epilogue(t, zero_set, nvis, nkept + t.ctr[cs + 2], lane, seq);
-  back_range<FREE, PROFILE, MULTI, SAFEDIV, LZ, SPH>(c, m, t, f, L, trunc_threshold, nvis, gw, nw, lane, tile, depth_raw, rgb_raw, deferred, want_stamp);
-  if (FREE) {
+  const int nvis = h.ctr[cs + 0];
+  const int ncfree = FREE ? h.ctr[cs + 2] : 0;
+  const int nkept = h.ctr[cs + 1];
+  if (gw == 0) frame_epilogue(h.ctr, ((ColdRef) h.cold)->t.h_levels, zero_set, nvis, nkept + h.ctr[cs + 2], lane, seq);
+  back_range<FREE, PROFILE, MULTI, SAFEDIV, LZ, SPH>(c, m, h, L, trunc_threshold, nvis, gw, nw, lane, tile, depth_raw, rgb_raw, deferred, want_stamp);
+  if (FREE && gw * (LZ ? kWave : 1) < ncfree) {
+    const Tab t = cold_tab(h.cold);
+    const Fast f = cold_fast(h.cold, h.dcx, h.want);
     if (LZ) free_candidates<PROFILE, LZ>(t, f, L, trunc_threshold, ncfree, gw, nw, lane, want_stamp);
     else free_range<PROFILE, MULTI>(t, L, ncfree, gw, nw, lane, deferred);
   }
 }
 
 template <bool FREE, bool PROFILE, bool MULTI, bool SAFEDIV, int LZ = 0, bool SPH = false>
-__global__ __launch_bounds__(256) void k_back(const Cam c, const Map m, const Tab t, const Fast f, const Lists L, const int set, const int zero_set,
+__global__ __launch_bounds__(256) void k_back(const Cam c, const Map m, const BackHot h, const Lists L, const int set, const int zero_set,
                                               const float trunc_threshold, const float* __restrict__ depth_raw,
                                               const uint8_t* __restrict__ rgb_raw, u32* __restrict__ deferred, const u32 want_stamp, const int seq) {
   extern __shared__ __attribute__((aligned(16))) uint2 s_tile[];
   const int wpw = blockDim.x >> 6;
-  back_role<FREE, PROFILE, MULTI, SAFEDIV, LZ, SPH>(c, m, t, f, L, set, zero_set, trunc_threshold, depth_raw, rgb_raw, deferred, blockIdx.x * wpw + (threadIdx.x >> 6),
-                                               gridDim.x * wpw, threadIdx.x & 63, &s_tile[(threadIdx.x >> 6) * kTileMaxPx], want_stamp, seq);
+  back_role<FREE, PROFILE, MULTI, SAFEDIV, LZ, SPH>(c, m, h, L, set, zero_set, trunc_threshold, depth_raw, rgb_raw, deferred, blockIdx.x * wpw + (threadIdx.x >> 6),
+                                               gridDim.x * wpw, threadIdx.x & 63, &s_tile[(threadIdx.x >> 6) * kTilePlane], want_stamp, seq);
 }
 
 __global__ __launch_bounds__(256) void k_reclaim(const Tab t, const Fast f) {
diff --git a/mrhash_amd/csrc/mrh_frame.h b/mrhash_amd/csrc/mrh_frame.h
--- a/mrhash_amd/csrc/mrh_frame.h
+++ b/mrhash_amd/csrc/mrh_frame.h
@@ -120,36 +120,52 @@
 }
 
 struct BackArgs {
-  Cam c; Map m; Tab t; Fast f; Lists L;
+  Cam c; Map m; BackHot h; Lists L;
   int set, zero_set;
   float thr;
   const float* depth_raw; const uint8_t* rgb_raw; u32* deferred;
   u32 want_stamp; int seq;
 };
 struct FrontArgs {
-  Cam c; Map m; Tab t; Fast f; Lists L;
+  Cam c; Map m; FrontHot h; Lists L;
   const float* depth; const uint8_t* rgb;
   int tiles_x, n_tiles; u32 stamp; int set, gc_on; float thr;
   int n_refill, low_blocks_to_allocate; const int* refill_flag;
 };
+BackHot back_hot(const mrh_ctx* c, const Fast& f) {
+  BackHot h = {};
+  h.pool = c->tab.pool; h.ctr = c->tab.ctr; h.dcx = f.dcx; h.summary = f.summary; h.want = f.want; h.cold = c->d_cold;
+#ifdef MRH_TRACE
+  h.trace = f.trace;
+#endif
+  return h;
+}
+FrontHot front_hot(const mrh_ctx* c, const Fast& f) {
+  FrontHot h = {};
+  h.keys = c->tab.keys; h.slot_mask = c->tab.slot_mask; h.max_probe = c->tab.max_probe; h.ctr = c->tab.ctr; h.dcx = f.dcx; h.want = f.want; h.cold = c->d_cold;
+#ifdef MRH_TRACE
+  h.trace = f.trace;
+#endif
+  return h;
+}
 BackArgs back_args(const mrh_ctx* c, const FramePlan& p, const Cam& k, const Fast& f, const Lists& L) {
-  if (p.kind == FRAME_FUSED_MR) return {k, c->map, c->tab, f, L, p.set, p.zero_set, p.gc_thr, c->d_depth, c->d_rgb, (u32*) c->d_reint, 0u, 0};
-  return {k, c->map, c->tab, f, L, p.set, p.zero_set, p.gc_thr, nullptr, nullptr, nullptr, p.stamp, p.seq};
+  if (p.kind == FRAME_FUSED_MR) return {k, c->map, back_hot(c, f), L, p.set, p.zero_set, p.gc_thr, c->d_depth, c->d_rgb, (u32*) c->d_reint, 0u, 0};
+  return {k, c->map, back_hot(c, f), L, p.set, p.zero_set, p.gc_thr, nullptr, nullptr, nullptr, p.stamp, p.seq};
 }
 int refill_wgs(const mrh_ctx* c) { return (c->low_blocks_to_allocate + 255) / 256; }
 FrontArgs front_args(const mrh_ctx* c, const FramePlan& p, const Cam& k, const Fast& f, const Lists& L) {
   const int gc_on = p.max_num_frames > 0 ? 1 : 0;
   if (p.kind == FRAME_FUSED_MR)
-    return {k, c->map, c->tab, f, L, c->d_depth, c->d_rgb, p.tiles_x, p.n_tiles, p.stamp, p.set, gc_on, p.gc_thr, refill_wgs(c), c->low_blocks_to_allocate, c->d_flag};
-  return {k, c->map, c->tab, f, L, c->d_depth, c->d_rgb, p.tiles_x, p.n_tiles, p.stamp, p.set, gc_on, p.gc_thr, 0, 0, nullptr};
+    return {k, c->map, front_hot(c, f), L, c->d_depth, c->d_rgb, p.tiles_x, p.n_tiles, p.stamp, p.set, gc_on, p.gc_thr, refill_wgs(c), c->low_blocks_to_allocate, c->d_flag};
+  return {k, c->map, front_hot(c, f), L, c->d_depth, c->d_rgb, p.tiles_x, p.n_tiles, p.stamp, p.set, gc_on, p.gc_thr, 0, 0, nullptr};
 }
 
 template <bool FREE, bool PROFILE, bool MULTI, bool SAFEDIV, int LZ, bool SPH>
 void back_as(const int grid, hipStream_t s, const EvPair* ev, const BackArgs& a) {
-  const size_t lds = (size_t) 4 * kTileMaxPx * sizeof(uint2);
+  const size_t lds = (size_t) 4 * kTilePlane * sizeof(uint2);
   if (ev) hipExtLaunchKernelGGL((k_back<FREE, PROFILE, MULTI, SAFEDIV, LZ, SPH>), dim3(grid), dim3(256), (uint32_t) lds, s, ev->a, ev->b, 0u,
-                                a.c, a.m, a.t, a.f, a.L, a.set, a.zero_set, a.thr, a.depth_raw, a.rgb_raw, a.deferred, a.want_stamp, a.seq);
-  else k_back<FREE, PROFILE, MULTI, SAFEDIV, LZ, SPH><<<grid, 256, lds, s>>>(a.c, a.m, a.t, a.f, a.L, a.set, a.zero_set, a.thr, a.depth_raw, a.rgb_raw,
+                                a.c, a.m, a.h, a.L, a.set, a.zero_set, a.thr, a.depth_raw, a.rgb_raw, a.deferred, a.want_stamp, a.seq);
+  else k_back<FREE, PROFILE, MULTI, SAFEDIV, LZ, SPH><<<grid, 256, lds, s>>>(a.c, a.m, a.h, a.L, a.set, a.zero_set, a.thr, a.depth_raw, a.rgb_raw,
                                                                              a.deferred, a.want_stamp, a.seq);
 }
 template <bool FREE, bool PROFILE, int LZ>
@@ -176,9 +192,9 @@
 
 template <bool PROFILE, bool MULTI, bool LAZY, bool SPH>
 void front_as(const int grid, hipStream_t s, const EvPair* ev, const FrontArgs& a) {
-  if (ev) hipExtLaunchKernelGGL((k_front<PROFILE, MULTI, LAZY, SPH>), dim3(grid), dim3(256), 0, s, ev->a, ev->b, 0u, a.c, a.m, a.t, a.f, a.L, a.depth, a.rgb,
+  if (ev) hipExtLaunchKernelGGL((k_front<PROFILE, MULTI, LAZY, SPH>), dim3(grid), dim3(256), 0, s, ev->a, ev->b, 0u, a.c, a.m, a.h, a.L, a.depth, a.rgb,
                                 a.tiles_x, a.n_tiles, a.stamp, a.set, a.gc_on, a.thr, a.n_refill, a.low_blocks_to_allocate, a.refill_flag);
-  else k_front<PROFILE, MULTI, LAZY, SPH><<<grid, 256, 0, s>>>(a.c, a.m, a.t, a.f, a.L, a.depth, a.rgb, a.tiles_x, a.n_tiles, a.stamp, a.set, a.gc_on, a.thr,
+  else k_front<PROFILE, MULTI, LAZY, SPH><<<grid, 256, 0, s>>>(a.c, a.m, a.h, a.L, a.depth, a.rgb, a.tiles_x, a.n_tiles, a.stamp, a.set, a.gc_on, a.thr,
                                                                a.n_refill, a.low_blocks_to_allocate, a.refill_flag);
 }
 template <bool PROFILE>
@@ -387,9 +403,13 @@
   main_stream_changed_map(c);
   HIP_TRY(c, hipMemsetAsync(ps.want_ring, 0, (size_t) kPipeRing * c->slots * sizeof(u32), c->stream));
   if (!ps.h_levels) HIP_TRY(c, pinned_alloc(c, ps.h_levels, 4 * sizeof(int)));
-  HIP_TRY(c, hipStreamCreateWithFlags(&ps.stream_front, hipStreamNonBlocking));
   ps.h_levels[0] = (int) c->num_blocks - 1; ps.h_levels[1] = 0; ps.h_levels[2] = -1;
   c->tab.h_levels = ps.h_levels;
+  {
+    const int rc = publish_cold(c);
+    if (rc) return rc;
+  }
+  HIP_TRY(c, hipStreamCreateWithFlags(&ps.stream_front, hipStreamNonBlocking));
   return MRH_OK;
 }
 
```

After: 27850 frames/s, median of 5. 1.5% higher.
